# trailofbits/reverie

Measured on AMD Instinct MI355X. Metric: prover AND-gates/sec on GF(2) Bristol circuit; 1/2/4/8-GPU; proof bit-exact, higher is better.
Workload: dtype u32; 1 GPU; synthetic layered AND/XOR GF(2) circuit, 10027008 gates (5014185 AND), 4096 inputs, 153 layers x 65536, p_and=0.5, 256 reps x 8 players, 40 online; parallelism=reps/1, levels=163, compile_hint=RV_COMPILE_WHOLE_PROVER, gate_stream_bytes=334698564

## Files before the change

reverie_amd/csrc/batch.inc:

```

static int replay_recorded(rv_ctx* ctx, std::vector<LaunchRecorder>& recs, std::vector<void*>& pinned_tmp, std::vector<void*>& device_tmp) {
    const size_t batch = recs.size(), n = recs[0].calls.size();
    for (size_t b = 1; b < batch; b++)
        if (recs[b].calls.size() != n) return RV_E_DEVICE;
    size_t total = 0;
    std::vector<size_t> off(n, 0);
    for (size_t i = 0; i < n; i++) {
        const auto& c0 = recs[0].calls[i];
        for (size_t b = 1; b < batch; b++) {
            const auto& c = recs[b].calls[i];
            if (c.replay != c0.replay || c.fill != c0.fill || c.grid.x != c0.grid.x || c.block.x != c0.block.x || c.arg_bytes != c0.arg_bytes) return RV_E_DEVICE;
        }
        if (!c0.replay) continue;
        if (c0.grid.y != 1 || c0.grid.z != 1) return RV_E_DEVICE;
        off[i] = total;
        total += ((size_t)c0.arg_bytes * batch + 15) & ~(size_t)15;
    }
    uint8_t* d_args = nullptr;
    if (total) {
        uint8_t* h = (uint8_t*)g_pinned.get(std::max<size_t>(total, PinnedPool::MIN_BYTES));
        if (!h) return RV_E_NOMEM;
        pinned_tmp.push_back(h);
        for (size_t i = 0; i < n; i++) {
            const uint32_t ab = recs[0].calls[i].arg_bytes;
            if (!recs[0].calls[i].replay) continue;
            for (size_t b = 0; b < batch; b++) memcpy(h + off[i] + b * ab, recs[b].calls[i].args.data(), ab);
        }
        int r = dalloc(ctx, total, &d_args);
        if (r) return r;
        device_tmp.push_back(d_args);
        if (hipMemcpyAsync(d_args, h, total, hipMemcpyHostToDevice, ctx->stream) != hipSuccess) return RV_E_DEVICE;
    }
    for (size_t i = 0; i < n; i++) {
        const auto& c0 = recs[0].calls[i];
        if (c0.replay) {
            c0.replay(ctx->stream, c0.grid, c0.block, d_args + off[i], (unsigned)batch);
        } else {
            for (size_t b = 0; b < batch; b++) {
                const auto& c = recs[b].calls[i];
                if ((c.fill ? hipMemsetAsync(c.dst, c.value, c.n, ctx->stream) : hipMemcpyAsync(c.dst, c.src, c.n, c.kind, ctx->stream)) != hipSuccess)
                    return RV_E_DEVICE;
            }
        }
    }
    if (hipGetLastError() != hipSuccess) return RV_E_DEVICE;
    for (auto& r : recs) r.calls.clear();
    return RV_OK;
}

static size_t batch_big_gates() {
    static const size_t n = [] {
        const char* e = getenv("RV_BATCH_BIG_GATES");
        return e ? (size_t)strtoull(e, nullptr, 10) : (size_t)1 << 20;
    }();
    return n;
}

static void launch_levels_batched(rv_ctx* ctx, const rv_circuit* c, int mode, const InterpParams* d_pp, const Interp64Params* d_pp64, size_t batch) {
    const Compiled& cc = c->cc;
    const bool has64 = !cc.gates64.empty();
    const size_t n_levels = cc.level_start.empty() ? 0 : cc.level_start.size() - 1;
    for (size_t l = 0; l < n_levels; l++) {
        if (lds_run_for_batch(c, l, batch)) {
            const auto& pl = c->lds_runs[(size_t)c->lds_run_of_level[l]];
            if (l == pl.run.l0) {
                launch_interp_lds(ctx->stream, mode, pl.qs, RV_TOTAL_REPS / 4, c->d_lds_recs + pl.run.rec0, pl.run.n_steps, pl.run.n_slots,
                                  pl.run.eo0, pl.run.ep0, InterpParams{}, d_pp, (uint32_t)batch);
                if (has64) ctx->count();
            }
            continue;
        }
        if (c->run_of_level[l] >= 0) {
            const auto& run = c->narrow_runs[(size_t)c->run_of_level[l]];
            if (l == run.first) {
                launch_interp_narrow_batched(ctx->stream, c->d_gates, c->d_level_range, run.first, run.second, run.tiny, d_pp, (uint32_t)batch, mode);
                if (has64) ctx->count();
            }
            continue;
        }
        launch_interp_batched(ctx->stream, c->d_gates, cc.level_range[l], d_pp, (uint32_t)batch, mode);
        if (has64 && cc.level_start[l + 1] > cc.level_start[l]) ctx->count();
        if (has64 && cc.level_start64[l + 1] > cc.level_start64[l]) {
            launch_interp64_batched(ctx->stream, mode, c->d_gates64, cc.level_start64[l], cc.level_start64[l + 1], d_pp64, (uint32_t)batch);
            ctx->count();
        }
    }
}

struct BatchDst {
    uint8_t** proofs;
    size_t* proof_lens;
    uint8_t* d_dst;
    size_t stride;
};

static int prove_framed_device(rv_ctx* ctx, const rv_circuit* c, const WitSrc& w, const uint8_t* seeds, uint8_t* d_dst) {
    rv_shard* s = nullptr;
    int rc = rv_shard_commit_impl(ctx, c, w, seeds, 0, RV_TOTAL_REPS, &s, true);
    if (rc) return rc;
    do {
        void* d = nullptr;
        size_t lens[4];
        if ((rc = shard_open_impl(s, nullptr, d_dst, &d, lens, true, nullptr, nullptr, true))) break;
        int err = 0;
        if (!launch_frame_counts(ctx->stream, d_dst, 0, 1, lens) || hipGetLastError() != hipSuccess) {
            rc = RV_E_DEVICE;
            break;
        }
        if (hipMemcpyAsync(&err, s->d_err, sizeof err, hipMemcpyDeviceToHost, ctx->stream) != hipSuccess ||
            hipStreamSynchronize(ctx->stream) != hipSuccess) {
            rc = hip_fail(hipGetLastError(), "rv_prove_batch_device", __FILE__, __LINE__);
            break;
        }
        ctx->collect();
        if (err) rc = RV_E_WITNESS_INVALID;
    } while (0);
    rv_shard_destroy(s);
    return rc;
}

static int rv_prove_batch_impl(rv_ctx* ctx, const rv_circuit* c, size_t batch, const WitSrc& w, const uint8_t* seeds, const BatchDst& out) {
    LibBusy busy_guard;
    const uint8_t* const wit_gf2 = w.gf2;
    const uint64_t* const wit_z64 = w.z64;
    const size_t n_gf2 = w.n_gf2, n_z64 = w.n_z64;
    uint8_t** const proofs = out.proofs;
    size_t* const proof_lens = out.proof_lens;
    const bool dev = out.d_dst != nullptr;
    if (!ctx || !c || !batch || (dev ? !seeds : (!proofs || !proof_lens))) return RV_E_ARG;
    const Compiled& cc = c->cc;
    for (size_t b = 0; b < batch && !dev; b++) proofs[b] = nullptr, proof_lens[b] = 0;
    if (n_gf2 < cc.n_in || n_z64 < cc.n_in64) return RV_E_WITNESS_SHORT;
    if ((cc.n_in && !wit_gf2) || (cc.n_in64 && !wit_z64)) return RV_E_ARG;
    std::vector<uint8_t> os_seeds;
    if (!seeds) {
        os_seeds.resize(batch * RV_TOTAL_REPS * 16);
        size_t got = 0;
        while (got < os_seeds.size()) {
            ssize_t n = getrandom(os_seeds.data() + got, os_seeds.size() - got, 0);
            if (n <= 0) return RV_E_DEVICE;
            got += (size_t)n;
        }
        seeds = os_seeds.data();
    }
    auto one_by_one = [&]() {
        for (size_t b = 0; b < batch && dev; b++) {
            int rc = prove_framed_device(ctx, c, w.from(b), seeds + b * RV_TOTAL_REPS * 16, out.d_dst + b * out.stride);
            if (rc) return rc;
        }
        if (dev) return (int)RV_OK;
        for (size_t b = 0; b < batch; b++) {
            int rc = guarded([&]() -> int { return rv_prove_impl(ctx, c, w.from(b), seeds + b * RV_TOTAL_REPS * 16, &proofs[b], &proof_lens[b]); });
            if (rc) {
                for (size_t k = 0; k <= b; k++) rv_free(proofs[k]), proofs[k] = nullptr, proof_lens[k] = 0;
                return rc;
            }
        }
        return (int)RV_OK;
    };
    if (batch == 1) return one_by_one();
    HIPCHK(hipSetDevice(ctx->device));
    const size_t big_gates = batch_big_gates();
    const bool has64 = !cc.gates64.empty();
    if (has64 && cc.gates.size() + cc.gates64.size() >= big_gates) return one_by_one();
    if (has64) {
        size_t free_b = 0, total_b = 0;
        if (hipMemGetInfo(&free_b, &total_b) != hipSuccess) return RV_E_DEVICE;
        uint8_t om[RV_TOTAL_REPS];
        for (uint32_t r = 0; r < RV_TOTAL_REPS; r++) om[r] = r < RV_ONLINE_REPS ? 0 : RV_PLAYERS;
        const size_t per_proof = cc.info.scratch_bytes + open_layout(cc, om, RV_TOTAL_REPS, true).total + cc.n_in + 8 * cc.n_in64 + 4096;
        size_t chunk = std::min<size_t>(std::max<size_t>((free_b + ctx->cached_bytes) / 2 / per_proof, 2), 4096);
        if (const char* e = getenv("RV_BATCH_MAX")) chunk = std::min<size_t>(chunk, (size_t)std::max(atoi(e), 1));
        if (batch > chunk) {
            for (size_t b0 = 0; b0 < batch; b0 += chunk) {
                const int rc = rv_prove_batch_impl(ctx, c, std::min(chunk, batch - b0), w.from(b0), seeds + b0 * RV_TOTAL_REPS * 16,
                                                   dev ? BatchDst{nullptr, nullptr, out.d_dst + b0 * out.stride, out.stride}
                                                       : BatchDst{proofs + b0, proof_lens + b0, nullptr, 0});
                if (rc) {
                    for (size_t k = 0; k < b0 && !dev; k++) rv_free(proofs[k]), proofs[k] = nullptr, proof_lens[k] = 0;
                    return rc;
                }
            }
            return RV_OK;
        }
    }
    if (dev && cc.gates.size() >= big_gates) return one_by_one();
    if (cc.gates.size() >= big_gates) {
        constexpr size_t T_MAX = 8;
        static const size_t T = [] {
            const char* e = getenv("RV_BATCH_THREADS");
            return (size_t)std::min(std::max(e ? atoi(e) : 3, 1), (int)T_MAX);
        }();
        static const std::string classes = [] {
            const char* e = getenv("RV_BATCH_CLASSES");
            return std::string(e ? e : "HLHLHLHLHLHLHLHL");
        }();
        static const int prio_levels = [] {
            int lo = 0, hi = 0;
            if (hipDeviceGetStreamPriorityRange(&lo, &hi) != hipSuccess) lo = hi = 0, (void)hipGetLastError();
            return lo - hi + 1;
        }();
        auto cls = [&](size_t i) {
            const char ch = i < classes.size() ? classes[i] : 'N';
            const int lowest = prio_levels - 1;
            return prio_levels < 2 ? -1 : ch == 'H' ? 0 : ch == 'L' ? lowest : lowest / 2 + (lowest == 1 ? -1 : 0);
        };
        while (ctx->workers.size() < T) {
            rv_ctx* w = nullptr;
            const size_t k = ctx->workers.size();
            int mc = cls(2 * k), kc = cls(2 * k + 1);
            if (mc < 0 && kc >= 0) mc = kc;
            int rcw = ctx_create_impl(ctx->device, &w, mc, kc);
            if (rcw) return rcw;
            ctx->workers.push_back(w);
        }
        uint8_t canon[RV_TOTAL_REPS];
        for (uint32_t r = 0; r < RV_TOTAL_REPS; r++) canon[r] = r < RV_ONLINE_REPS ? 0 : RV_PLAYERS;
        const size_t stride = (open_layout(cc, canon, RV_TOTAL_REPS, true).total + 4095) & ~(size_t)4095;
        uint8_t* slab = (uint8_t*)g_pinned.get(std::max<size_t>(stride * batch, PinnedPool::MIN_BYTES));
        if (!slab) return RV_E_NOMEM;
        int rcs[T_MAX] = {};
        std::thread th[T_MAX];
        static const bool big_stats = getenv("RV_BATCH_STATS") != nullptr;
        const auto t_call = std::chrono::steady_clock::now();
        std::vector<std::array<double, 5>> span(batch);
        std::atomic<size_t> next_proof{0};
        for (size_t t = 0; t < T; t++)
            th[t] = std::thread([&, t] {
                try {
                    if (hipSetDevice(ctx->device) != hipSuccess) {
                        rcs[t] = RV_E_DEVICE;
                        return;
                    }
                    for (size_t b; rcs[t] == RV_OK && (b = next_proof.fetch_add(1, std::memory_order_relaxed)) < batch;) {
                        span[b][0] = std::chrono::duration<double, std::milli>(std::chrono::steady_clock::now() - t_call).count();
                        rcs[t] = rv_prove_impl(ctx->workers[t], c, WitSrc{w.from(b).gf2, n_gf2, w.stride_gf2, nullptr, 0, 0, w.dev},
                                               seeds + b * RV_TOTAL_REPS * 16, &proofs[b], &proof_lens[b], slab + b * stride, stride);
                        span[b][1] = std::chrono::duration<double, std::milli>(std::chrono::steady_clock::now() - t_call).count();
                        for (int k = 0; k < 3; k++) span[b][2 + k] = g_prove_marks[k];
                        if (big_stats && g_prove_marks[1] > 5.0) {
                            std::string line = "[rv batch] slow host side, proof " + std::to_string(b) + ":";
                            for (auto& m : g_ht.marks) line += std::string(" ") + m.first + " " + std::to_string(m.second).substr(0, 5);
                            fprintf(stderr, "%s\n", line.c_str());
                        }
                    }
                } catch (...) {
                    rcs[t] = RV_E_NOMEM;
                }
            });
        for (size_t t = 0; t < T; t++) th[t].join();
        if (big_stats) {
            fprintf(stderr, "[rv batch] %zu proofs on %zu workers, %.2f ms:", batch, T,
                    std::chrono::duration<double, std::milli>(std::chrono::steady_clock::now() - t_call).count());
            for (size_t b = 0; b < batch; b++)
                fprintf(stderr, " %zu[%.1f-%.1f: q %.1f o %.1f s %.1f]", b, span[b][0], span[b][1], span[b][2], span[b][3], span[b][4]);
            fprintf(stderr, "\n");
        }
        for (int r : rcs)
            if (r) {
                for (size_t b = 0; b < batch; b++) proofs[b] = nullptr, proof_lens[b] = 0;
                g_pinned.put(slab);
                return r;
            }
        g_pinned.share(slab, batch);
        ctx->prof.calls += batch;
        return RV_OK;
    }
    std::vector<rv_shard*> sh(batch, nullptr);
    std::vector<InterpParams> pp(batch);
    std::vector<Interp64Params> pp64(has64 ? batch : 0);
    InterpParams* d_pp = nullptr;
    int rc = RV_OK;
    uint8_t* staging = nullptr;
    std::vector<void*> pinned_tmp;
    std::vector<void*> device_tmp;
    auto cleanup = [&](int code) {
        g_recorder = nullptr;
        (void)hipStreamSynchronize(ctx->stream);
        for (rv_shard* s : sh)
            if (s) {
                s->destroy();
                delete s;
            }
        ctx->release(d_pp);
        for (void* q : device_tmp) ctx->release(q);
        for (void* q : pinned_tmp) g_pinned.put(q);
        if (staging) g_pinned.put(staging);
        if (code && !dev)
            for (size_t b = 0; b < batch; b++) rv_free(proofs[b]), proofs[b] = nullptr, proof_lens[b] = 0;
        return code;
    };
    const uint32_t R = RV_TOTAL_REPS;
    std::vector<LaunchRecorder> recs(batch);
    for (auto& r : recs) r.batch = (unsigned)batch;
    struct RecorderOff {
        ~RecorderOff() { g_recorder = nullptr; }
    } recorder_off;
    static const bool stats = getenv("RV_BATCH_STATS") != nullptr;
    auto t_last = std::chrono::steady_clock::now();
    auto mark = [&](const char* what) {
        if (!stats) return;
        const auto t = std::chrono::steady_clock::now();
        fprintf(stderr, "[rv batch] %-28s %8.3f ms\n", what, std::chrono::duration<double, std::milli>(t - t_last).count());
        t_last = t;
    };
    auto replay = [&]() -> int { return replay_recorded(ctx, recs, pinned_tmp, device_tmp); };
    constexpr size_t SLAB_HEAD = 256;
    const size_t wit_stride = (std::max<size_t>(cc.n_in, 1) + 15) & ~(size_t)15;
    uint8_t canon[RV_TOTAL_REPS];
    for (uint32_t r = 0; r < RV_TOTAL_REPS; r++) canon[r] = r < RV_ONLINE_REPS ? 0 : RV_PLAYERS;
    const size_t out_stride = (open_layout(cc, canon, R, true).total + 4 + 255) & ~(size_t)255;
    uint8_t *d_seeds_all = nullptr, *d_wit_all = nullptr, *d_out_all = nullptr;
    int* d_err_all = nullptr;
    if ((rc = dalloc(ctx, SLAB_HEAD + batch * (size_t)R * 16, &d_seeds_all))) return cleanup(rc);
    device_tmp.push_back(d_seeds_all);
    if ((rc = dalloc(ctx, SLAB_HEAD + batch * wit_stride, &d_wit_all))) return cleanup(rc);
    device_tmp.push_back(d_wit_all);
    if (!dev) {
        if ((rc = dalloc(ctx, SLAB_HEAD + batch * out_stride, &d_out_all))) return cleanup(rc);
        device_tmp.push_back(d_out_all);
    }
    if ((rc = dalloc(ctx, SLAB_HEAD / sizeof(int) + batch, &d_err_all))) return cleanup(rc);
    device_tmp.push_back(d_err_all);
    if (hipMemcpyAsync(d_seeds_all + SLAB_HEAD, seeds, batch * (size_t)R * 16, hipMemcpyHostToDevice, ctx->stream) != hipSuccess ||
        (cc.n_in && hipMemcpy2DAsync(d_wit_all + SLAB_HEAD, wit_stride, wit_gf2, w.stride_gf2, cc.n_in, batch, w.kind(),
                                     ctx->stream) != hipSuccess))
        return cleanup(RV_E_DEVICE);
    const size_t wit64_stride = (std::max<size_t>(cc.n_in64, 1) + 1) & ~(size_t)1;
    uint64_t* d_wit64_all = nullptr;
    if (has64) {
        if ((rc = dalloc(ctx, SLAB_HEAD / 8 + batch * wit64_stride, &d_wit64_all))) return cleanup(rc);
        device_tmp.push_back(d_wit64_all);
        if (cc.n_in64 && hipMemcpy2DAsync(d_wit64_all + SLAB_HEAD / 8, wit64_stride * 8, wit_z64, w.stride_z64 * 8, cc.n_in64 * 8, batch,
                                          w.kind(), ctx->stream) != hipSuccess)
            return cleanup(RV_E_DEVICE);
    }
    wit_count(w, batch * (cc.n_in + cc.n_in64 * 8));
    for (size_t b = 0; b < batch && !rc; b++) {
        rv_shard* s = sh[b] = new rv_shard();
        s->ctx = ctx;
        s->c = c;
        s->rep_begin = 0;
        s->R = R;
        s->NQ = R / 4;
        s->d_seeds = d_seeds_all + SLAB_HEAD + b * (size_t)R * 16;
        s->d_wit = d_wit_all + SLAB_HEAD + b * wit_stride;
        s->d_err = d_err_all + SLAB_HEAD / sizeof(int) + b;
        if ((rc = dalloc(ctx, (size_t)R * 128, &s->d_keys))) break;
        g_recorder = &recs[b];
        launch_expand_seeds(ctx->stream, s->d_seeds, R, s->d_keys);
        Interp64Params p64{};
        pp[b] = InterpParams{};
        pp[b].wit = s->d_wit;
        if (!(rc = shard_setup_prg(s, nullptr))) rc = shard_run_alloc(s, pp[b], p64);
        if (has64) {
            p64.wit = d_wit64_all + SLAB_HEAD / 8 + b * wit64_stride;
            pp64[b] = p64;
        }
        g_recorder = nullptr;
    }
    if (rc) return cleanup(rc);
    mark("record setup/masks");
    ctx->phase(RV_PH_MASKS);
    if ((rc = replay())) return cleanup(rc);
    mark("replay setup/masks");
    ctx->phase(RV_PH_INTERP);
    if ((rc = dalloc(ctx, batch, &d_pp))) return cleanup(rc);
    if (hipMemcpyAsync(d_pp, pp.data(), batch * sizeof(InterpParams), hipMemcpyHostToDevice, ctx->stream) != hipSuccess) return cleanup(RV_E_DEVICE);
    Interp64Params* d_pp64 = nullptr;
    if (has64) {
        if ((rc = dalloc(ctx, batch, &d_pp64))) return cleanup(rc);
        device_tmp.push_back(d_pp64);
        if (hipMemcpyAsync(d_pp64, pp64.data(), batch * sizeof(Interp64Params), hipMemcpyHostToDevice, ctx->stream) != hipSuccess) return cleanup(RV_E_DEVICE);
    }
    launch_levels_batched(ctx, c, MODE_PROVE, d_pp, d_pp64, batch);
    if (has64) ctx->phase(-1);
    mark("interpreter launches");
    size_t slot = 0;
    size_t lens[4] = {0, 0, 0, 0};
    for (size_t b = 0; b < batch && !rc; b++) {
        rv_shard* s = sh[b];
        void* d = nullptr;
        g_recorder = &recs[b];
        if (!(rc = shard_run_hash(s)) && !(rc = shard_join(s)))
            rc = shard_open_impl(s, nullptr, dev ? out.d_dst + b * out.stride : d_out_all + SLAB_HEAD + b * out_stride, &d, lens, true, nullptr, nullptr, true);
        g_recorder = nullptr;
    }
    if (rc) return cleanup(rc);
    mark("record digests/openings");
    ctx->phase(RV_PH_HASH);
    if ((rc = replay())) return cleanup(rc);
    ctx->phase(-1);
    mark("replay digests/openings");
    const size_t total = 32 + 4 * 8 + lens[0] + lens[1] + lens[2] + lens[3];
    if (dev) {
        if (total > out.stride || batch > 0x3FFFFFFFu || !launch_frame_counts(ctx->stream, out.d_dst, out.stride, (uint32_t)batch, lens) ||
            hipGetLastError() != hipSuccess)
            return cleanup(RV_E_DEVICE);
        staging = (uint8_t*)g_pinned.get(std::max<size_t>(batch * sizeof(int), PinnedPool::MIN_BYTES));
        if (!staging) return cleanup(RV_E_NOMEM);
        if (hipMemcpyAsync(staging, d_err_all + SLAB_HEAD / sizeof(int), batch * sizeof(int), hipMemcpyDeviceToHost, ctx->stream) != hipSuccess)
            return cleanup(RV_E_DEVICE);
    } else {
        if (total > out_stride) return cleanup(RV_E_DEVICE);
        slot = out_stride;
        staging = (uint8_t*)g_pinned.get(std::max<size_t>(slot * batch + batch * sizeof(int), PinnedPool::MIN_BYTES));
        if (!staging) return cleanup(RV_E_NOMEM);
        if (hipMemcpyAsync(staging, d_out_all + SLAB_HEAD, slot * batch, hipMemcpyDeviceToHost, ctx->stream) != hipSuccess ||
            hipMemcpyAsync(staging + slot * batch, d_err_all + SLAB_HEAD / sizeof(int), batch * sizeof(int), hipMemcpyDeviceToHost,
                           ctx->stream) != hipSuccess)
            return cleanup(RV_E_DEVICE);
        for (size_t b = 0; b < batch; b++) proof_lens[b] = total;
    }
    mark("queue device-to-host copies");
    if (hipStreamSynchronize(ctx->stream) != hipSuccess) return cleanup(hip_fail(hipGetLastError(), "batch sync", __FILE__, __LINE__));
    ctx->collect();
    mark("wait for the GPU");
    for (size_t b = 0; b < batch; b++) {
        int err = 0;
        memcpy(&err, staging + slot * batch + b * sizeof(int), sizeof err);
        if (err) return cleanup(RV_E_WITNESS_INVALID);
    }
    if (!dev) {
        static const bool copy_out = getenv("RV_BATCH_COPY_OUT") != nullptr;
        const uint64_t counts[4] = {RV_ONLINE_REPS, RV_PREPROCESSING_REPS, RV_ONLINE_REPS, RV_PREPROCESSING_REPS};
        if (copy_out) {
            for (size_t b = 0; b < batch; b++) {
                proofs[b] = (uint8_t*)malloc(proof_lens[b]);
                if (!proofs[b]) return cleanup(RV_E_NOMEM);
                memcpy(proofs[b], staging + b * slot, proof_lens[b]);
            }
        } else {
            g_pinned.share(staging, batch);
            for (size_t b = 0; b < batch; b++) proofs[b] = staging + b * slot;
            staging = nullptr;
        }
        for (size_t b = 0; b < batch; b++) {
            size_t off = 32;
            for (int k = 0; k < 4; k++) {
                put_le64(proofs[b] + off, counts[k]);
                off += 8 + lens[k];
            }
        }
    }
    ctx->prof.calls += batch;
    mark("copy proofs out");
    rc = cleanup(RV_OK);
    mark("cleanup");
    return rc;
}

extern "C" int rv_prove_batch(rv_ctx* ctx, const rv_circuit* c, size_t batch, const uint8_t* wit_gf2, size_t n_gf2,
                              const uint64_t* wit_z64, size_t n_z64, const uint8_t* seeds, uint8_t** proofs, size_t* proof_lens) {
    try {
        return rv_prove_batch_impl(ctx, c, batch, wit_host(wit_gf2, n_gf2, wit_z64, n_z64), seeds, BatchDst{proofs, proof_lens, nullptr, 0});
    } catch (...) {
        g_last_error = "out of host memory";
        return RV_E_NOMEM;
    }
}
```

reverie_amd/csrc/gf2dev.h:

```cpp
#pragma once
#include <hip/hip_runtime.h>
#include <stdint.h>

namespace rv {

__device__ __forceinline__ uint32_t smear01(uint32_t t) {
    uint32_t r;
    asm("v_lshlrev_b32 %0, 8, %1\n\tv_sub_u32 %0, %0, %1" : "=&v"(r) : "v"(t));
    return r;
}
__device__ __forceinline__ uint32_t recon32(uint32_t t) {
    t ^= t >> 4;
    t ^= t >> 2;
    t ^= t >> 1;
    t &= 0x01010101u;
    return smear01(t);
}

__device__ __forceinline__ uint32_t expand4(uint32_t n) {
    const uint32_t t = (n | (n << 7) | (n << 14) | (n << 21)) & 0x01010101u;
    return smear01(t);
}
__device__ __forceinline__ uint32_t compress4(uint32_t x) {
    const uint32_t y = x & 0x08040201u;
    return (y | (y >> 8) | (y >> 16) | (y >> 24)) & 0xFu;
}
__device__ __forceinline__ uint32_t load_bits(const uint8_t* base, size_t row, uint32_t NQ, uint32_t q) {
    return expand4(((uint32_t)base[row * (NQ >> 1) + (q >> 1)] >> (4 * (q & 1))) & 0xFu);
}
__device__ __forceinline__ uint32_t pair_swap(uint32_t v) {
    return (uint32_t)__builtin_amdgcn_mov_dpp((int)v, 0xB1, 0xF, 0xF, true);
}
__device__ __forceinline__ void store_bits(uint8_t* base, size_t row, uint32_t NQ, uint32_t q, uint32_t smeared) {
    const uint32_t n = compress4(smeared);
    const uint32_t other = pair_swap(n);
    if (!(q & 1)) base[row * (NQ >> 1) + (q >> 1)] = (uint8_t)(n | (other << 4));
}

}
```

reverie_amd/csrc/internal.h:

```cpp
#pragma once
#include <hip/hip_runtime.h>
#include <stddef.h>
#include <stdint.h>

#include "../../include/reverie_amd.h"

namespace rv {


constexpr int RV_LIN_K = 3;
struct Gate {
    uint32_t op;
    uint32_t dst;
    uint32_t m;
    uint32_t eo;
    uint32_t ep;
    uint32_t x;
    uint32_t a[RV_LIN_K], b[RV_LIN_K];
};

enum GateOp : uint32_t {
    G_INPUT = 0,
    G_XORK,
    G_MUL,
    G_ASSERT,
    G_RANDOM,
    G_RECON
};
__host__ __device__ inline uint32_t g_op(const Gate& g) { return g.op & 0xFFu; }
__host__ __device__ inline uint32_t g_na(const Gate& g) { return (g.op >> 8) & 0xFu; }
__host__ __device__ inline uint32_t g_nb(const Gate& g) { return (g.op >> 12) & 0xFu; }
__host__ __device__ inline uint32_t g_ca(const Gate& g) { return (g.op >> 16) & 1u; }
__host__ __device__ inline uint32_t g_cb(const Gate& g) { return (g.op >> 17) & 1u; }

struct Gate64 {
    uint32_t op;
    uint32_t dst;
    uint32_t a, b;
    uint32_t m;
    uint32_t m2;
    uint64_t eo;
    uint64_t ep;
    uint32_t x;
    uint32_t xc;
    uint64_t imm;
    uint32_t am, bm;
};
constexpr uint32_t G64_MASK_ROW = 0x80000000u;

enum Gate64Op : uint32_t {
    G64_INPUT = 0, G64_ADD, G64_SUB, G64_ADDC, G64_SUBC, G64_MULC, G64_MUL, G64_ASSERT, G64_RANDOM, G64_CONST, G64_B2A
};

struct Interp64Params {
    uint32_t R;
    uint64_t* wmask;
    uint64_t* wcorr;
    const uint64_t* masks;
    uint64_t* on;
    uint64_t* pre;
    uint64_t on_words, pre_words;
    const uint64_t* wit;
    const uint8_t* omit;
    const uint64_t* sup_in;
    const uint64_t* sup_corr;
    const uint64_t* sup_rec;
    uint32_t sup_r;
    const uint8_t* corr2;
    const uint32_t* masks2;
    uint32_t NQ;
    int* err;
};

enum Mode : int { MODE_PROVE = 0, MODE_VERIFY = 1, MODE_PROVE_V = 2, MODE_VERIFY_C = 4 };
constexpr int RV_DEV_ZERO_CHECK = 0x100;

struct InterpParams {
    uint32_t NQ;
    uint32_t* rows;
    uint8_t* corr;
    uint32_t* on;
    uint8_t* pre;
    uint8_t* vclr;
    uint64_t* vc;
    const uint8_t* wit;
    const uint32_t* on_mask;
    const uint32_t* sup_in;
    const uint32_t* sup_corr;
    const uint32_t* sup_rec;
    uint32_t sup_nq;
    int* err;
};

void set_device_lds_limit(size_t bytes);
size_t device_lds_limit();

struct EvalParams {
    uint32_t B, W;
    uint32_t* val;
    const uint32_t* win;
    uint64_t* v64;
    const uint64_t* wz;
    uint64_t wz_stride;
    uint32_t* n_failed;
    uint32_t* first2;
    uint32_t* first64;
};
struct WireForm {
    uint32_t b[RV_LIN_K];
    uint32_t c;
};
void launch_eval_level(hipStream_t st, const EvalParams& p, const Gate* d_gates, uint32_t lo, uint32_t n2, const Gate64* d_gates64, uint32_t lo64,
                       uint32_t n64);
struct LevelRange;
void launch_eval_walk(hipStream_t st, const EvalParams& p, const Gate* d_gates, const LevelRange* d_lr, const Gate64* d_gates64, const uint32_t* d_ls64,
                      uint32_t n_levels, uint32_t S, uint32_t threads);
void launch_eval_wit(hipStream_t st, const uint8_t* d_wit , size_t stride, uint32_t n, uint32_t B, uint32_t W,
                     uint32_t* d_out );
void launch_eval_out(hipStream_t st, const EvalParams& p, const WireForm* d_forms, uint32_t n_gf2, const uint32_t* d_ssa64, uint32_t n_z64,
                     uint8_t* d_out2 , uint64_t* d_out64 );

struct EvalFold {
    const uint32_t* rec2;
    const uint64_t* op2;
    const uint32_t* rec64;
    const uint64_t* op64;
    uint32_t n2, n64;
    uint64_t op_base;
    uint64_t* first_op;
    uint64_t* total;
};
void launch_eval_fold(hipStream_t st, const EvalParams& p, const EvalFold& f);
void launch_eval_out_sel(hipStream_t st, const EvalParams& p, const WireForm* d_forms, const uint32_t* d_sel2, uint32_t n_sel2, const uint32_t* d_ssa64,
                         const uint32_t* d_sel64, uint32_t n_sel64, uint8_t* d_out2 , uint64_t* d_out64 );
void launch_eval_status(hipStream_t st, const EvalParams& p, const EvalFold& f, rv_eval_status* d_out );
void launch_eval_stream_out(hipStream_t st, const EvalParams& p, uint32_t n_gf2, uint32_t n_z64, uint32_t b0, uint32_t nb, uint8_t* d_out2,
                            uint64_t* d_out64);

void launch_expand_seeds(hipStream_t st, const uint8_t* d_seeds, uint32_t n_reps, uint8_t* d_keys );
constexpr uint32_t RK_BYTES = 208;
constexpr uint32_t RK_AREAS = 13;
constexpr uint64_t RV_MAX_CTR_BLOCKS = 1ull << 24;
void launch_key_schedule(hipStream_t st, const uint8_t* d_keys, uint32_t n_slots, uint8_t* d_rkbytes );
void launch_setup_keys(hipStream_t st, const uint8_t* d_seeds, uint32_t NQ, uint8_t* d_keys, uint8_t* d_rkbytes, uint32_t* d_rk, uint32_t* d_img);
void launch_bitslice_rk(hipStream_t st, const uint8_t* d_rkbytes, uint32_t NQ, uint32_t* d_rk );
void launch_aes_gf2_masks(hipStream_t st, const uint32_t* d_rk, const uint32_t* d_keep, uint32_t NQ, uint64_t first_block,
                          uint64_t n_blocks, uint32_t* d_masks);
bool aes_col4_supports(uint32_t NQ);
size_t aes_col4_image_bytes(uint32_t NQ);
void launch_rk_col4(hipStream_t st, const uint32_t* d_rk, uint32_t NQ, uint32_t* d_img);
void launch_aes_gf2_masks_col4(hipStream_t st, const uint32_t* d_img, const uint32_t* d_keep, uint32_t NQ, uint64_t first_block, uint64_t n_blocks,
                               uint32_t* d_masks);
void launch_aes_blocks(hipStream_t st, const uint8_t* d_rkbytes, uint32_t n_keys, uint64_t first_block, uint64_t n_blocks,
                       uint8_t* d_out);
struct LevelRange {
    uint32_t lo, mul11, mul, xor2, xork, hi;
};
bool any_level_general(const LevelRange* lr, size_t n_levels);
void launch_interp(hipStream_t st, int mode, const Gate* d_gates, const LevelRange& r, const InterpParams& p,
                   const LevelRange* next = nullptr);
void launch_interp_narrow(hipStream_t st, int mode, const Gate* d_gates, const LevelRange* d_level_range, uint32_t l0, uint32_t l1,
                          int tiny, const InterpParams& p);
void launch_interp_batched(hipStream_t st, const Gate* d_gates, const LevelRange& r, const InterpParams* d_pp, uint32_t batch,
                           int mode = MODE_PROVE);
bool b3_pair_big_ok(uint64_t n_pre, uint64_t n_on, uint32_t NQ, const uint32_t* d_quads = nullptr, uint32_t n_quads = 0);
uint32_t launch_b3_pair_big(hipStream_t st, const uint8_t* d_pre, uint64_t n_pre, const uint32_t* d_on, uint64_t n_on, uint32_t NQ, uint32_t* cv_a0,
                            uint32_t* cv_a1, uint32_t* cv_b0, uint32_t* cv_b1, uint32_t* d_dig_pre, uint32_t* d_dig_on, const uint32_t* d_quads = nullptr,
                            uint32_t n_quads = 0);
bool launch_b3_pair_small(hipStream_t st, const uint8_t* d_pre, uint64_t n_pre, const uint32_t* d_on, uint64_t n_on, uint32_t NQ, uint32_t* d_cv_a,
                          uint32_t* d_cv_b, uint32_t* d_dig_pre, uint32_t* d_dig_on, const uint32_t* d_quads = nullptr, uint32_t n_quads = 0);
void launch_store_word(hipStream_t st, const int* d_src, int* dst_mapped);
void launch_pack_corr_all(hipStream_t st, const uint8_t* d_bits, uint64_t n_items, uint64_t byte0, uint64_t n_bytes, uint64_t pitch, uint8_t* d_out);
struct OpenDirect {
    uint32_t n_direct = 0, tile = 0;
    uint64_t rvec_at = 0, rvec_len = 0;
};
void launch_copy_gaps(hipStream_t st, const uint8_t* d_img, uint8_t* dst_mapped, uint64_t total, uint64_t first, uint64_t rec, uint64_t corr_at,
                      uint64_t corr_len, uint32_t n_rec, const uint8_t* d_omit , uint32_t rep_limit, OpenDirect od = OpenDirect(),
                      const int* d_err = nullptr, int* err_dst_mapped = nullptr );
uint32_t extract_tile_bytes(uint64_t n_items);
uint32_t extract_from_bits_tile_bytes(uint64_t n_items);
void launch_publish(hipStream_t st, const uint32_t* d_src, uint32_t n_words, uint32_t* dst_mapped, uint32_t* flag_mapped, uint32_t seq);
void launch_store_words(hipStream_t st, const uint32_t* d_src, uint32_t n_words, uint32_t* dst_mapped, const int* d_err, int* dst_err_mapped);
bool launch_frame_counts(hipStream_t st, uint8_t* d_out, uint64_t stride, uint32_t batch, const size_t lens[4]);
struct LdsRec;
void launch_interp_lds(hipStream_t st, int mode, uint32_t QS, uint32_t NQ, const LdsRec* d_recs, uint32_t n_steps, uint32_t n_slots,
                       uint32_t eo0, uint32_t ep0, const InterpParams& p, const InterpParams* d_pp, uint32_t batch);
void launch_interp_narrow_batched(hipStream_t st, const Gate* d_gates, const LevelRange* d_level_range, uint32_t l0, uint32_t l1,
                                  int tiny, const InterpParams* d_pp, uint32_t batch, int mode = MODE_PROVE);
void launch_interp64(hipStream_t st, int mode, const Gate64* d_gates, uint32_t lo, uint32_t hi, const Interp64Params& p);
void launch_interp64_batched(hipStream_t st, int mode, const Gate64* d_gates, uint32_t lo, uint32_t hi, const Interp64Params* d_pp, uint32_t batch);
void launch_aes_z64_masks(hipStream_t st, const uint32_t* d_rk, const uint32_t* d_keep, uint32_t NQ, uint64_t n_blocks,
                          uint64_t* d_masks64, uint64_t first_block = 0);
struct Z64FLevel {
    uint32_t mul0, mul1, lin1, oth1;
};
struct Z64FParams {
    const uint32_t* rk;
    uint32_t NQ;
    uint64_t* wmask;
    uint64_t* masks;
    uint64_t* on;
    uint64_t* pre;
    uint64_t on_words, pre_words;
    const uint64_t* wit;
    uint64_t* v;
    int* err;
    uint64_t first_block;
    uint32_t qg0, qgn;
    const uint8_t* omit;
    const uint32_t* keep;
    uint64_t* wcorr;
    const uint64_t* sup_in;
    const uint64_t* sup_corr;
    const uint64_t* sup_rec;
    uint32_t sup_r;
};
bool z64_fused_supports(uint32_t NQ);
uint32_t z64_fused_qw(uint32_t NQ);
void launch_z64_fused(hipStream_t st, const Gate64* d_gates, const Z64FLevel& lv, const Z64FParams& p);
uint32_t launch_b3_contig(hipStream_t st, const uint64_t* d_streams, uint64_t n_words, uint32_t R, uint32_t* d_cv_a, uint32_t* d_cv_b,
                      uint32_t* d_digest);
void launch_extract64(hipStream_t st, const uint64_t* d_stream, uint64_t stride_words, const uint64_t* d_offs ,
                      uint64_t n_items, int add_omit, uint32_t R, const uint8_t* d_omit, const uint64_t* d_dst_off, uint8_t* d_out,
                      const struct OnlineList* d_ol = nullptr ,
                      uint32_t rep_min = 0 );
void launch_unpack64(hipStream_t st, const uint8_t* d_blob, const uint64_t* d_src_off, const uint64_t* d_src_len,
                     const uint8_t* d_omit, uint64_t n_items, uint32_t R, uint64_t* d_out, uint32_t out_r );
uint32_t launch_b3_stream(hipStream_t st, const uint32_t* d_stream, uint64_t n_events, uint32_t NQ, uint32_t* d_cv_a,
                      uint32_t* d_cv_b, uint32_t* d_digest , const uint32_t* d_quads = nullptr, uint32_t n_quads = 0);
uint32_t launch_b3_stream_bits(hipStream_t st, const uint8_t* d_stream, uint64_t n_events, uint32_t NQ, uint32_t* d_cv_a,
                           uint32_t* d_cv_b, uint32_t* d_digest);
size_t b3_stream_scratch_words(uint64_t n_events, uint32_t R);
void launch_b3_stream_chunks(hipStream_t st, const uint32_t* d_stream, uint64_t n_events, uint32_t NQ, uint32_t* d_cv, const uint32_t* d_quads,
                             uint32_t n_quads, uint64_t chunk_base, uint32_t root_ok);
void launch_b3_stream_bits_chunks(hipStream_t st, const uint8_t* d_stream, uint64_t n_events, uint32_t NQ, uint32_t* d_cv, uint64_t chunk_base,
                                  uint32_t root_ok);
void launch_b3_contig_chunks(hipStream_t st, const uint64_t* d_streams, uint64_t stride_words, uint64_t n_words, uint32_t R, uint32_t* d_cv,
                             uint64_t chunk_base, uint32_t root_ok);
void launch_b3_pairs(hipStream_t st, const uint32_t* d_pending, const uint32_t* d_in, uint64_t n_pairs, uint32_t R, uint32_t* d_out);
struct B3PairsBatch {
    static constexpr uint32_t MAX = 32;
    const uint32_t* pending[MAX];
    const uint32_t* in[MAX];
    uint32_t* out[MAX];
    uint32_t n;
};
void launch_b3_pairs_batched(hipStream_t st, const B3PairsBatch& L, uint64_t n_pairs, uint32_t R);
struct B3FoldList {
    uint32_t n;
    const uint32_t* p[48];
};
void launch_b3_fold(hipStream_t st, const B3FoldList& L, const uint32_t* d_last, uint32_t R, uint32_t* d_digest);
uint32_t b3_reduce_tree(hipStream_t st, uint32_t* cur, uint32_t* nxt, uint64_t n, uint32_t R, uint32_t* d_digest);
void launch_join(hipStream_t st, const uint32_t* d_pre2, const uint32_t* d_on2, const uint32_t* d_pre64, const uint32_t* d_on64,
                 uint32_t R, uint8_t* d_h );
struct OnlineList {
    uint32_t n;
    uint32_t rep[RV_ONLINE_REPS];
    uint64_t dst[RV_ONLINE_REPS];
};
void launch_extract_from_bits(hipStream_t st, const uint8_t* d_bits, uint64_t n_items, uint32_t NQ,
                              const OnlineList* d_ol , uint8_t* d_out, uint32_t rep_min = 0 );
struct FsLayout {
    uint64_t base[4];
    uint64_t sz2, sz64, l2r, l2c, l64r, l64c;
    uint32_t framed;
    uint8_t* comm2;
};
void launch_fs_challenge(hipStream_t st, const uint8_t* d_h, const FsLayout& L, uint32_t rep_begin, uint32_t R, uint8_t* d_comm,
                         uint8_t* d_omit, uint8_t* d_omit_all, uint64_t* d_offs, OnlineList* d_ol, uint32_t* d_res,
                         uint32_t* mbox = nullptr ,
                         uint32_t* mbox_flag = nullptr, uint32_t mbox_seq = 0);
bool launch_open_small(hipStream_t st, uint32_t R, const uint8_t* d_omit, const uint8_t* d_seeds, const uint8_t* d_keys, const uint32_t* d_on2,
                       const uint32_t* d_on64, const uint64_t* d_offs, uint64_t l2r, uint64_t l2c, uint64_t l2i, uint64_t l64r, uint64_t l64c, uint64_t l64i,
                       const uint32_t* d_on, const uint32_t* d_rec_rows, uint64_t n_rec, const uint8_t* d_pre, uint64_t n_pre, const uint32_t* d_in_rows,
                       uint64_t n_in, uint32_t NQ, const OnlineList* d_ol, uint32_t corr_rep_min, uint8_t* d_out, const int* d_err, int* err_dst_mapped,
                       bool heads_inputs_only = false);
void launch_extract_bits(hipStream_t st, const void* d_stream, const uint32_t* d_rows , uint64_t n_items,
                         uint32_t NQ, int kind, const uint8_t* d_omit, const uint64_t* d_dst_off, uint8_t* d_out, uint8_t* d_out2 = nullptr,
                         uint32_t n_direct = 0);
void launch_unpack_bits(hipStream_t st, const uint8_t* d_blob, const uint64_t* d_src_off, const uint64_t* d_src_len,
                        const uint8_t* d_omit, uint64_t n_items, uint32_t NQ, int kind, uint32_t* d_rows_out, uint32_t out_nq ,
                        uint64_t first_item = 0 );
void launch_shard_init(hipStream_t st, int* d_err, uint32_t* d_zero_mask, uint32_t n_mask_words , uint8_t* d_zero_corr,
                       uint32_t n_corr_bytes , uint32_t* d_fill = nullptr , uint32_t n_fill_rows = 0,
                       const uint32_t* digest = nullptr, uint8_t* d_zero_byte = nullptr );
void launch_fill_digests(hipStream_t st, uint32_t* d_dst, uint32_t n_rows, const uint32_t digest[8]);
void launch_overlay_rows(hipStream_t st, uint32_t* d_dst, const uint32_t* d_src, const uint8_t* d_omit, uint32_t R,
                         uint32_t row_words, int want_online);
void launch_hook_recon_gf2(hipStream_t st, const uint64_t* d_shares, uint64_t n, uint64_t* d_out);
void launch_hook_recon_z64(hipStream_t st, const uint64_t* d_shares , uint64_t n, uint64_t* d_out );
void launch_open_headers(hipStream_t st, uint32_t R, const uint8_t* d_omit, const uint8_t* d_seeds, const uint8_t* d_keys,
                         const uint32_t* d_on2, const uint32_t* d_on64, const uint64_t* d_off2, const uint64_t* d_off64,
                         uint64_t lens2_rec, uint64_t lens2_corr, uint64_t lens2_in, uint64_t lens64_rec, uint64_t lens64_corr,
                         uint64_t lens64_in, uint8_t* d_out);


}
```

reverie_amd/csrc/interp.hip:

```cpp
#include <stdlib.h>

#include <algorithm>

#include "gf2dev.h"
#include "internal.h"
#include "launch.h"

namespace rv {

static size_t g_device_lds_limit = 160 * 1024;
void set_device_lds_limit(size_t bytes) { g_device_lds_limit = bytes; }
size_t device_lds_limit() { return g_device_lds_limit; }


__device__ __forceinline__ uint32_t gather_rows(const uint32_t* rows, const uint32_t* ids, uint32_t NQ, uint32_t q) {
    uint32_t v = 0;
#pragma unroll
    for (int i = 0; i < RV_LIN_K; i++) v ^= rows[(size_t)ids[i] * NQ + q];
    return v;
}
__device__ __forceinline__ uint32_t gather_corr_byte(const uint8_t* corr, const uint32_t* ids, uint32_t NQ, uint32_t o) {
    uint32_t v = 0;
#pragma unroll
    for (int i = 0; i < RV_LIN_K; i++) v ^= corr[(size_t)ids[i] * (NQ >> 1) + o];
    return v;
}
__device__ __forceinline__ uint32_t gather_corr(const uint8_t* corr, const uint32_t* ids, uint32_t NQ, uint32_t q) {
    return (gather_corr_byte(corr, ids, NQ, q >> 1) >> (4 * (q & 1))) & 0xFu;
}

__device__ __forceinline__ uint32_t gather_vclr(const uint8_t* vclr, const uint32_t* ids) {
    uint32_t v = 0;
#pragma unroll
    for (int i = 0; i < RV_LIN_K; i++) v ^= vclr[ids[i]];
    return v;
}

__device__ __forceinline__ uint32_t vc_nib(uint64_t c, uint32_t q) {
    const uint32_t w = (q & 8) ? (uint32_t)(c >> 32) : (uint32_t)c;
    return q < 16 ? (w >> (4 * (q & 7))) & 0xFu : 0u;
}
__device__ __forceinline__ uint64_t gather_vc(const uint64_t* vc, const uint32_t* ids) {
    uint64_t v = 0;
#pragma unroll
    for (int i = 0; i < RV_LIN_K; i++) v ^= vc[ids[i]];
    return v;
}
__device__ __forceinline__ void vc_store(uint64_t* vc, size_t row, uint32_t q, uint32_t smeared) {
    uint32_t v = q < 16 ? compress4(smeared) << (4 * (q & 7)) : 0u;
    v |= (uint32_t)__builtin_amdgcn_update_dpp(0, (int)v, 0x111, 0xF, 0xF, true);
    v |= (uint32_t)__builtin_amdgcn_update_dpp(0, (int)v, 0x112, 0xF, 0xF, true);
    v |= (uint32_t)__builtin_amdgcn_update_dpp(0, (int)v, 0x114, 0xF, 0xF, true);
    if (q == 7 || q == 15) ((uint32_t*)(vc + row))[q >> 3] = v;
}
constexpr bool is_verify(int mode) { return mode == MODE_VERIFY || mode == MODE_VERIFY_C; }

template <int MODE>
__device__ __forceinline__ void interp_one(const Gate& g, const InterpParams& p, uint32_t NQ, uint32_t q, uint32_t onm) {
    switch (g_op(g)) {
    case G_INPUT: {
        const uint32_t lam = p.rows[(size_t)g.m * NQ + q];
        uint32_t corr;
        if (!is_verify(MODE)) {
            const uint32_t w = p.wit[g.x] ? 0xFFFFFFFFu : 0u;
            corr = w ^ recon32(lam);
        } else {
            corr = onm ? (p.sup_in[(size_t)g.x * p.sup_nq + q] & onm) : 0u;
        }
        if (!is_verify(MODE) || onm) p.on[(size_t)g.eo * NQ + q] = corr;
        if (MODE == MODE_PROVE_V) {
            if (q == 0) p.vclr[g.dst] = p.wit[g.x] ? 1 : 0;
        } else if (MODE == MODE_VERIFY_C) {
            vc_store(p.vc, g.dst, q, corr);
        } else {
            store_bits(p.corr, g.dst, NQ, q, corr);
        }
        break;
    }
    case G_XORK: {
        p.rows[(size_t)g.dst * NQ + q] = gather_rows(p.rows, g.a, NQ, q) ^ gather_rows(p.rows, g.b, NQ, q);
        if (MODE == MODE_PROVE_V) {
            if (q == 0) p.vclr[g.dst] = (uint8_t)((g_ca(g) ^ gather_vclr(p.vclr, g.a) ^ gather_vclr(p.vclr, g.b)) & 1u);
            break;
        }
        if (MODE == MODE_VERIFY_C) {
            if (q == 0) p.vc[g.dst] = gather_vc(p.vc, g.a) ^ gather_vc(p.vc, g.b) ^ (g_ca(g) ? ~0ull : 0ull);
            break;
        }
        if (!(q & 1)) {
            const size_t h = NQ >> 1, o = q >> 1;
            const uint32_t c = (g_ca(g) ? 0xFFu : 0u) ^ gather_corr_byte(p.corr, g.a, NQ, o) ^ gather_corr_byte(p.corr, g.b, NQ, o);
            p.corr[(size_t)g.dst * h + o] = (uint8_t)c;
        }
        break;
    }
    case G_RANDOM: {
        if (MODE == MODE_VERIFY_C) {
            if (q == 0) p.vc[g.dst] = 0;
            break;
        }
        if (!(q & 1)) p.corr[(size_t)g.dst * (NQ >> 1) + (q >> 1)] = 0;
        break;
    }
    case G_MUL: {
        const uint32_t lx = gather_rows(p.rows, g.a, NQ, q), ly = gather_rows(p.rows, g.b, NQ, q);
        const uint32_t lab = p.rows[(size_t)g.m * NQ + q], lnew = p.rows[(size_t)(g.m + 1) * NQ + q];
        const uint32_t a = recon32(lx), b = recon32(ly), c = recon32(lab);
        uint32_t cx, cy, vx = 0, vy = 0;
        if (MODE == MODE_PROVE_V) {
            vx = (gather_vclr(p.vclr, g.a) ^ g_ca(g)) & 1u;
            vy = (gather_vclr(p.vclr, g.b) ^ g_cb(g)) & 1u;
            cx = a ^ (vx ? 0xFFFFFFFFu : 0u);
            cy = b ^ (vy ? 0xFFFFFFFFu : 0u);
        } else if (MODE == MODE_VERIFY_C) {
            cx = expand4(vc_nib(gather_vc(p.vc, g.a), q)) ^ (g_ca(g) ? 0xFFFFFFFFu : 0u);
            cy = expand4(vc_nib(gather_vc(p.vc, g.b), q)) ^ (g_cb(g) ? 0xFFFFFFFFu : 0u);
        } else {
            cx = expand4(gather_corr(p.corr, g.a, NQ, q)) ^ (g_ca(g) ? 0xFFFFFFFFu : 0u);
            cy = expand4(gather_corr(p.corr, g.b, NQ, q)) ^ (g_cb(g) ? 0xFFFFFFFFu : 0u);
        }
        uint32_t delta = (a & b) ^ c;
        uint32_t s = (ly & cx) ^ (lx & cy) ^ lab ^ lnew;
        uint32_t r;
        if (!is_verify(MODE)) {
            r = recon32(s);
        } else {
            if (onm) {
                delta = (p.sup_corr[(size_t)g.ep * p.sup_nq + q] & onm) | (delta & ~onm);
                s ^= p.sup_rec[(size_t)g.x * p.sup_nq + q];
            }
            r = recon32(s) & onm;
        }
        if (!is_verify(MODE) || onm) p.on[(size_t)g.eo * NQ + q] = s;
        store_bits(p.pre, g.ep, NQ, q, delta);
        if (MODE == MODE_PROVE_V) {
            if (q == 0) p.vclr[g.dst] = (uint8_t)(vx & vy);
        } else if (MODE == MODE_VERIFY_C) {
            vc_store(p.vc, g.dst, q, r ^ delta ^ (cx & cy));
        } else {
            store_bits(p.corr, g.dst, NQ, q, r ^ delta ^ (cx & cy));
        }
        break;
    }
    case G_RECON: {
        uint32_t m = gather_rows(p.rows, g.a, NQ, q);
        if (is_verify(MODE) && onm) m ^= p.sup_rec[(size_t)g.x * p.sup_nq + q];
        if (MODE == MODE_PROVE || onm) p.on[(size_t)g.eo * NQ + q] = m;
        uint32_t r = recon32(m);
        if (is_verify(MODE)) r &= onm;
        const uint32_t cx = expand4(gather_corr(p.corr, g.a, NQ, q)) ^ (g_ca(g) ? 0xFFFFFFFFu : 0u);
        p.rows[(size_t)g.dst * NQ + q] = 0;
        store_bits(p.corr, g.dst, NQ, q, r ^ cx);
        break;
    }
    case G_ASSERT: {
        uint32_t m = gather_rows(p.rows, g.a, NQ, q);
        if (is_verify(MODE) && onm) m ^= p.sup_rec[(size_t)g.x * p.sup_nq + q];
        if (!is_verify(MODE) || onm) p.on[(size_t)g.eo * NQ + q] = m;
        if (MODE == MODE_PROVE_V) {
            if (q == 0 && ((gather_vclr(p.vclr, g.a) ^ g_ca(g)) & 1u) != 0) atomicOr(p.err, RV_E_WITNESS_INVALID);
        } else {
            const uint32_t cx = expand4(MODE == MODE_VERIFY_C ? vc_nib(gather_vc(p.vc, g.a), q) : gather_corr(p.corr, g.a, NQ, q)) ^ (g_ca(g) ? 0xFFFFFFFFu : 0u);
            if (MODE == MODE_PROVE) {
                if ((recon32(m) ^ cx) != 0) atomicOr(p.err, RV_E_WITNESS_INVALID);
            } else {
                if (((recon32(m) ^ cx) & onm) != 0) atomicOr(p.err, RV_DEV_ZERO_CHECK);
            }
        }
        break;
    }
    default:
        break;
    }
}

template <int MODE>
__global__ __launch_bounds__(256) void k_interp(const Gate* __restrict__ gates, uint32_t lo, uint32_t hi, InterpParams p) {
    const uint32_t NQ = p.NQ;
    const uint32_t tid = blockIdx.x * blockDim.x + threadIdx.x;
    const uint32_t q = tid % NQ;
    const uint32_t worker = tid / NQ;
    const uint32_t n_workers = (gridDim.x * blockDim.x) / NQ;
    const uint32_t onm = (is_verify(MODE)) ? p.on_mask[q] : 0u;
    for (uint32_t gi = lo + worker; gi < hi; gi += n_workers) {
        const Gate g = gates[gi];
        interp_one<MODE>(g, p, NQ, q, onm);
    }
}

#ifndef RV_INTERP_UNROLL
#define RV_INTERP_UNROLL 4
#endif
#ifndef RV_INTERP_UNROLL_SMALL
#define RV_INTERP_UNROLL_SMALL 2
#endif
#ifndef RV_INTERP_UNROLL_MID
#define RV_INTERP_UNROLL_MID 4
#endif
#ifndef RV_INTERP_UNROLL_FAST
#define RV_INTERP_UNROLL_FAST 4
#endif
#ifndef RV_INTERP_UXOR_FAST
#define RV_INTERP_UXOR_FAST 0
#endif
__host__ __device__ constexpr int interp_unroll(int NQ, bool general = true) {
    return NQ >= 64 ? (general ? RV_INTERP_UNROLL : RV_INTERP_UNROLL_FAST) : NQ >= 32 ? RV_INTERP_UNROLL_MID : RV_INTERP_UNROLL_SMALL;
}

struct PfPlan {
    uint32_t dist;
    uint32_t rem;
    uint32_t n[2][4];
    uint32_t start[2][4];
};
template <uint32_t STEP>
__device__ __forceinline__ const Gate* pf_target(const Gate* __restrict__ gates, const PfPlan& pf, uint32_t t) {
    uint32_t tt = t + pf.dist;
#pragma unroll
    for (int k = 0; k < 2; k++) {
#pragma unroll
        for (int c = 0; c < 4; c++) {
            if (tt < pf.n[k][c]) return gates + pf.start[k][c] + tt * STEP;
            tt -= pf.n[k][c];
        }
        tt += pf.rem;
    }
    return nullptr;
}
template <uint32_t STEP>
__device__ __forceinline__ uint32_t pf_touch(const Gate* g, uint32_t lane) {
    constexpr uint32_t BYTES = STEP * (uint32_t)sizeof(Gate), NL = (BYTES + 127) / 128;
    uint32_t v = 0;
    if (g && lane <= NL) v = *(const uint32_t*)((const char*)g + (lane < NL ? lane * 128 : BYTES - 4));
    return v;
}
__device__ __forceinline__ void pf_sink(uint32_t v) { asm volatile("" ::"v"(v)); }

template <int MODE, int NQ, int U, int KA, int KB>
__device__ __forceinline__ void mulU(const Gate* __restrict__ gates, uint32_t g0, const InterpParams& p, uint32_t sub, uint32_t q,
                                     uint32_t onm, const Gate* pf = nullptr) {
    constexpr uint32_t GPW = 64 / NQ, H = NQ / 2;
    const bool on_wr = !is_verify(MODE) || ((__ballot(onm != 0) >> ((sub * NQ + q) & ~7u)) & 0xFFull) != 0;
    Gate g[U];
#pragma unroll
    for (int u = 0; u < U; u++) g[u] = gates[g0 + u * GPW + sub];
    uint32_t lx[U], ly[U], lab[U], lnew[U], bx[U], by[U], sc[U], sr[U];
    uint32_t ra[U][KA], ca[U][KA], rb[U][KB], cb[U][KB];
    const uint32_t* const vc32 = (const uint32_t*)p.vc + ((q >> 3) & 1u);
#pragma unroll
    for (int u = 0; u < U; u++) {
        const int na = (int)g_na(g[u]), nb = (int)g_nb(g[u]);
#pragma unroll
        for (int i = 0; i < KA; i++) {
            ra[u][i] = 0;
            ca[u][i] = 0;
            if (i == 0 || i < na) {
                ra[u][i] = p.rows[(size_t)g[u].a[i] * NQ + q];
                ca[u][i] = MODE == MODE_VERIFY_C ? vc32[2 * (size_t)g[u].a[i]]
                                                 : MODE == MODE_PROVE_V ? p.vclr[g[u].a[i]] : p.corr[(size_t)g[u].a[i] * H + (q >> 1)];
            }
        }
#pragma unroll
        for (int i = 0; i < KB; i++) {
            rb[u][i] = 0;
            cb[u][i] = 0;
            if (i == 0 || i < nb) {
                rb[u][i] = p.rows[(size_t)g[u].b[i] * NQ + q];
                cb[u][i] = MODE == MODE_VERIFY_C ? vc32[2 * (size_t)g[u].b[i]]
                                                 : MODE == MODE_PROVE_V ? p.vclr[g[u].b[i]] : p.corr[(size_t)g[u].b[i] * H + (q >> 1)];
            }
        }
        lab[u] = __builtin_nontemporal_load(&p.rows[(size_t)g[u].m * NQ + q]);
        lnew[u] = p.rows[(size_t)(g[u].m + 1) * NQ + q];
        if (is_verify(MODE)) {
            sc[u] = sr[u] = 0;
            if (onm) {
                sc[u] = p.sup_corr[(size_t)g[u].ep * p.sup_nq + q];
                sr[u] = p.sup_rec[(size_t)g[u].x * p.sup_nq + q];
            }
        }
    }
    const uint32_t pfv = pf_touch<U * GPW>(pf, sub * NQ + q);
#pragma unroll
    for (int u = 0; u < U; u++) {
        lx[u] = ra[u][0];
        bx[u] = ca[u][0];
        ly[u] = rb[u][0];
        by[u] = cb[u][0];
#pragma unroll
        for (int i = 1; i < KA; i++) {
            lx[u] ^= ra[u][i];
            bx[u] ^= ca[u][i];
        }
#pragma unroll
        for (int i = 1; i < KB; i++) {
            ly[u] ^= rb[u][i];
            by[u] ^= cb[u][i];
        }
    }
#pragma unroll
    for (int u = 0; u < U; u++) {
        const uint32_t a = recon32(lx[u]), b = recon32(ly[u]), c = recon32(lab[u]);
        uint32_t cx, cy;
        const uint32_t vx = (bx[u] ^ g_ca(g[u])) & 1u, vy = (by[u] ^ g_cb(g[u])) & 1u;
        if (MODE == MODE_PROVE_V) {
            cx = a ^ (vx ? 0xFFFFFFFFu : 0u);
            cy = b ^ (vy ? 0xFFFFFFFFu : 0u);
        } else if (MODE == MODE_VERIFY_C) {
            cx = expand4(q < 16 ? (bx[u] >> (4 * (q & 7))) & 0xFu : 0u) ^ (g_ca(g[u]) ? 0xFFFFFFFFu : 0u);
            cy = expand4(q < 16 ? (by[u] >> (4 * (q & 7))) & 0xFu : 0u) ^ (g_cb(g[u]) ? 0xFFFFFFFFu : 0u);
        } else {
            cx = expand4((bx[u] >> (4 * (q & 1))) & 0xFu) ^ (g_ca(g[u]) ? 0xFFFFFFFFu : 0u);
            cy = expand4((by[u] >> (4 * (q & 1))) & 0xFu) ^ (g_cb(g[u]) ? 0xFFFFFFFFu : 0u);
        }
        uint32_t delta = (a & b) ^ c;
        uint32_t s = (ly[u] & cx) ^ (lx[u] & cy) ^ lab[u] ^ lnew[u];
        uint32_t r = 0;
        if (MODE == MODE_PROVE) {
            r = recon32(s);
        } else if (is_verify(MODE)) {
            delta = (sc[u] & onm) | (delta & ~onm);
            s ^= sr[u];
            r = recon32(s) & onm;
        }
        if (!is_verify(MODE) || on_wr) __builtin_nontemporal_store(s, &p.on[(size_t)g[u].eo * NQ + q]);
        store_bits(p.pre, g[u].ep, NQ, q, delta);
        if (MODE == MODE_PROVE_V) {
            if (q == 0) p.vclr[g[u].dst] = (uint8_t)(vx & vy);
        } else if (MODE == MODE_VERIFY_C) {
            vc_store(p.vc, g[u].dst, q, r ^ delta ^ (cx & cy));
        } else {
            store_bits(p.corr, g[u].dst, NQ, q, r ^ delta ^ (cx & cy));
        }
    }
    pf_sink(pfv);
}

template <int MODE, int NQ, int U, int N>
__device__ __forceinline__ void xorU(const Gate* __restrict__ gates, uint32_t g0, const InterpParams& p, uint32_t sub, uint32_t q,
                                     const Gate* pf = nullptr) {
    constexpr uint32_t GPW = 64 / NQ, H = NQ / 2;
    Gate g[U];
#pragma unroll
    for (int u = 0; u < U; u++) g[u] = gates[g0 + u * GPW + sub];
    uint32_t x[U], bx[U], rr[U][N], cc[U][N];
#pragma unroll
    for (int u = 0; u < U; u++) {
        const int na = (int)g_na(g[u]), nb = (int)g_nb(g[u]);
#pragma unroll
        for (int i = 0; i < N; i++) {
            const uint32_t id = (N == 2) ? g[u].a[i] : (i < RV_LIN_K ? g[u].a[i] : g[u].b[i - RV_LIN_K]);
            rr[u][i] = 0;
            cc[u][i] = 0;
            if (N == 2 || (i < RV_LIN_K ? i < na : i - RV_LIN_K < nb)) {
                rr[u][i] = p.rows[(size_t)id * NQ + q];
                if (MODE == MODE_PROVE_V) {
                    if (q == 0) cc[u][i] = p.vclr[id];
                } else if (MODE == MODE_VERIFY_C) {
                    if (q < 2) cc[u][i] = ((const uint32_t*)p.vc)[2 * (size_t)id + q];
                } else if (q < H) {
                    cc[u][i] = p.corr[(size_t)id * H + q];
                }
            }
        }
    }
    const uint32_t pfv = pf_touch<U * GPW>(pf, sub * NQ + q);
#pragma unroll
    for (int u = 0; u < U; u++) {
        x[u] = 0;
        bx[u] = 0;
#pragma unroll
        for (int i = 0; i < N; i++) {
            x[u] ^= rr[u][i];
            bx[u] ^= cc[u][i];
        }
    }
#pragma unroll
    for (int u = 0; u < U; u++) {
        p.rows[(size_t)g[u].dst * NQ + q] = x[u];
        if (MODE == MODE_PROVE_V) {
            if (q == 0) p.vclr[g[u].dst] = (uint8_t)((bx[u] ^ g_ca(g[u])) & 1u);
        } else if (MODE == MODE_VERIFY_C) {
            if (q < 2) ((uint32_t*)p.vc)[2 * (size_t)g[u].dst + q] = bx[u] ^ (g_ca(g[u]) ? 0xFFFFFFFFu : 0u);
        } else if (q < H) {
            p.corr[(size_t)g[u].dst * H + q] = (uint8_t)(bx[u] ^ (g_ca(g[u]) ? 0xFFu : 0u));
        }
    }
    pf_sink(pfv);
}

template <int MODE, int NQ, bool GENERAL = true, bool PF = false, int UXOR = 0>
__device__ __forceinline__ void run_level(const Gate* __restrict__ gates, const LevelRange& r, const InterpParams& p, uint32_t wave,
                                          uint32_t n_waves, uint32_t lane, uint32_t onm, const Gate* pf_gates = nullptr,
                                          const PfPlan* pf = nullptr) {
    constexpr uint32_t GPW = 64 / NQ;
    const uint32_t q = lane % NQ, sub = lane / NQ;
    constexpr int U = interp_unroll(NQ, GENERAL);
    constexpr int UX = UXOR ? UXOR : U;
    static_assert(!PF || UX == U, "the prefetch plan assumes one step size");
    uint32_t slot = 0;
    auto my = [&](uint32_t used) { return (wave + n_waves - used % n_waves) % n_waves; };
    const uint32_t begin[5] = {r.lo, r.mul11, r.mul, r.xor2, r.xork}, end[5] = {r.mul11, r.mul, r.xor2, r.xork, r.hi};
    uint32_t rest[5];
#pragma unroll
    for (int c = 0; c < 4; c++) {
        const uint32_t STEP = (uint32_t)(c >= 2 ? UX : U) * GPW;
        const uint32_t n_full = (!GENERAL && (c == 1 || c == 3)) ? 0u : (end[c] - begin[c]) / STEP;
        rest[c] = begin[c] + n_full * STEP;
        for (uint32_t g0 = begin[c] + my(slot) * STEP; g0 < rest[c]; g0 += n_waves * STEP) {
            const Gate* t = nullptr;
            if (PF && pf->dist) t = pf_target<U * GPW>(pf_gates, *pf, slot + (g0 - begin[c]) / STEP);
            if (c == 0) mulU<MODE, NQ, U, 1, 1>(gates, g0, p, sub, q, onm, t);
            if (c == 1 && GENERAL) mulU<MODE, NQ, U, RV_LIN_K, RV_LIN_K>(gates, g0, p, sub, q, onm, t);
            if (c == 2) xorU<MODE, NQ, UX, 2>(gates, g0, p, sub, q, t);
            if (c == 3 && GENERAL) xorU<MODE, NQ, UX, 2 * RV_LIN_K>(gates, g0, p, sub, q, t);
        }
        slot += n_full;
    }
    rest[4] = begin[4];
    uint32_t cum[6];
    cum[0] = 0;
#pragma unroll
    for (int c = 0; c < 5; c++) cum[c + 1] = cum[c] + (end[c] - rest[c] + GPW - 1) / GPW;
    for (uint32_t t = my(slot); t < cum[5]; t += n_waves) {
        uint32_t c0 = rest[0], e0 = end[0], base = 0;
#pragma unroll
        for (int c = 1; c < 5; c++)
            if (t >= cum[c]) c0 = rest[c], e0 = end[c], base = cum[c];
        const uint32_t gi = c0 + (t - base) * GPW + sub;
        if (gi < e0) interp_one<MODE>(gates[gi], p, NQ, q, onm);
    }
}

template <int MODE, int NQ, bool GENERAL>
__global__ __launch_bounds__(256, MODE == MODE_VERIFY_C ? (GENERAL ? 4 : 7) : (GENERAL || NQ != 64) ? 1 : 8) void k_interp_full(const Gate* __restrict__ gates, LevelRange r, InterpParams p, PfPlan pf) {
    __builtin_amdgcn_s_setprio(1);
    const uint32_t lane = threadIdx.x & 63;
    const uint32_t wave = __builtin_amdgcn_readfirstlane((blockIdx.x * blockDim.x + threadIdx.x) >> 6);
    const uint32_t n_waves = gridDim.x * (blockDim.x >> 6);
    const uint32_t onm = (is_verify(MODE)) ? p.on_mask[lane % NQ] : 0u;
    constexpr int UXL = (!GENERAL && NQ == 64) ? RV_INTERP_UXOR_FAST : 0;
    constexpr bool PFL = UXL == 0 || UXL == interp_unroll(NQ, GENERAL);
    run_level<MODE, NQ, GENERAL, PFL, UXL>(gates, r, p, wave, n_waves, lane, onm, gates, &pf);
}

template <int MODE, int NQ>
__global__ __launch_bounds__(256) void k_interp_full_b(const Gate* __restrict__ gates, LevelRange r, const InterpParams* __restrict__ pp) {
    const InterpParams p = pp[blockIdx.y];
    const uint32_t lane = threadIdx.x & 63;
    const uint32_t wave = __builtin_amdgcn_readfirstlane((blockIdx.x * blockDim.x + threadIdx.x) >> 6);
    const uint32_t n_waves = gridDim.x * (blockDim.x >> 6);
    const uint32_t onm = (is_verify(MODE)) ? p.on_mask[lane % NQ] : 0u;
    run_level<MODE, NQ>(gates, r, p, wave, n_waves, lane, onm);
}

static bool level_is_general(const LevelRange& r) { return (r.mul - r.mul11) + (r.xork - r.xor2) >= 64; }

static uint32_t pf_dist(int NQ) {
    static const int env = [] {
        const char* e = getenv("RV_PF_DIST");
        return e ? atoi(e) : -1;
    }();
    const uint32_t v = env >= 0 ? (uint32_t)env : (NQ == 64 ? 4096u : 0u);
    return v & ~31u;
}

template <int NQ>
static PfPlan make_pf_plan(const LevelRange& r, const LevelRange* next) {
    constexpr uint32_t GPW = 64 / NQ;
    PfPlan pf{};
    pf.dist = pf_dist(NQ);
    if (!pf.dist) return pf;
    const LevelRange* lr[2] = {&r, next};
    uint32_t total = 0;
    for (int k = 0; k < 2; k++) {
        if (!lr[k]) break;
        const LevelRange& x = *lr[k];
        const bool general = level_is_general(x);
        const uint32_t step = (uint32_t)interp_unroll(NQ, general) * GPW;
        const uint32_t begin[4] = {x.lo, x.mul11, x.mul, x.xor2}, end[4] = {x.mul11, x.mul, x.xor2, x.xork};
        for (int c = 0; c < 4; c++) {
            pf.start[k][c] = begin[c];
            pf.n[k][c] = (!general && (c == 1 || c == 3)) ? 0u : (end[c] - begin[c]) / step;
            if (k == 0) total += pf.n[k][c];
        }
    }
    pf.rem = total & 31u;
    return pf;
}

template <int MODE, int NQ>
static void launch_interp_full_mode(hipStream_t st, dim3 grid, bool general, const Gate* d_gates, const LevelRange& r, const InterpParams& p,
                                    const PfPlan& pf) {
    if (general)
        hipLaunchKernelGGL((k_interp_full<MODE, NQ, true>), grid, dim3(256), 0, st, d_gates, r, p, pf);
    else
        hipLaunchKernelGGL((k_interp_full<MODE, NQ, false>), grid, dim3(256), 0, st, d_gates, r, p, pf);
}

template <int NQ>
static void launch_interp_full(hipStream_t st, int mode, const Gate* d_gates, const LevelRange& r, const InterpParams& p,
                               const LevelRange* next) {
    constexpr uint32_t GPW = 64 / NQ;
    const bool general = level_is_general(r);
    const PfPlan pf = make_pf_plan<NQ>(r, next);
    const uint32_t u = (uint32_t)interp_unroll(NQ, general);
    uint64_t waves = ((uint64_t)(r.hi - r.lo) + u * GPW - 1) / (u * GPW);
    uint64_t blocks = (waves + 3) / 4;
    if (blocks > 4096) blocks = 4096;
    if (blocks < 1) blocks = 1;
    const dim3 grid((unsigned)blocks);
    if (mode == MODE_PROVE_V) return launch_interp_full_mode<MODE_PROVE_V, NQ>(st, grid, general, d_gates, r, p, pf);
    if (mode == MODE_PROVE) return launch_interp_full_mode<MODE_PROVE, NQ>(st, grid, general, d_gates, r, p, pf);
    if constexpr (NQ == 64)
        if (mode == MODE_VERIFY_C) return launch_interp_full_mode<MODE_VERIFY_C, NQ>(st, grid, general, d_gates, r, p, pf);
    launch_interp_full_mode<MODE_VERIFY, NQ>(st, grid, general, d_gates, r, p, pf);
}


bool any_level_general(const LevelRange* lr, size_t n_levels) {
    for (size_t l = 0; l < n_levels; l++)
        if (level_is_general(lr[l])) return true;
    return false;
}

constexpr uint32_t NARROW_MAX_LEVELS = 1024;
constexpr uint32_t NARROW_WIN = 1024;
template <int MODE, int NQT, bool LEAN = false>
__device__ __forceinline__ void interp_narrow_body(const Gate* __restrict__ gates, const LevelRange* __restrict__ level_range,
                                                   uint32_t l0, uint32_t l1, const InterpParams& p) {
    __shared__ LevelRange s_lr[NARROW_MAX_LEVELS];
    __shared__ __attribute__((aligned(16))) Gate s_g[NARROW_WIN];
    const uint32_t NQ = NQT ? (uint32_t)NQT : p.NQ;
    const uint32_t lane = threadIdx.x & 63, wave = threadIdx.x >> 6;
    const uint32_t onm = (is_verify(MODE)) ? p.on_mask[NQT ? lane % NQ : threadIdx.x % NQ] : 0u;
    const uint32_t n_lv = l1 - l0;
    {
        const uint32_t* src = (const uint32_t*)(level_range + l0);
        uint32_t* dst = (uint32_t*)s_lr;
        for (uint32_t i = threadIdx.x; i < n_lv * (uint32_t)(sizeof(LevelRange) / 4); i += 1024) dst[i] = src[i];
    }
    __syncthreads();
    const uint32_t g_end = s_lr[n_lv - 1].hi;
    uint32_t win_lo = s_lr[0].lo, win_hi = win_lo;
    for (uint32_t l = 0; l < n_lv; l++) {
        const LevelRange r = s_lr[l];
        if (r.hi > win_hi) {
            win_lo = r.lo;
            win_hi = (r.lo + NARROW_WIN < g_end) ? r.lo + NARROW_WIN : g_end;
            const uint4* src = (const uint4*)(gates + win_lo);
            uint4* dst = (uint4*)s_g;
            for (uint32_t i = threadIdx.x; i < (win_hi - win_lo) * (uint32_t)(sizeof(Gate) / 16); i += 1024) dst[i] = src[i];
            __syncthreads();
        }
        const Gate* g = s_g - win_lo;
        if (NQT) {
            if (LEAN)
                run_level<MODE, NQT ? NQT : 64, false, false, 8>(g, r, p, wave, 16, lane, onm);
            else
                run_level<MODE, NQT ? NQT : 64>(g, r, p, wave, 16, lane, onm);
        } else {
            const uint32_t q = threadIdx.x % NQ, worker = threadIdx.x / NQ, n_workers = 1024 / NQ;
            for (uint32_t gi = r.lo + worker; gi < r.hi; gi += n_workers) interp_one<MODE>(g[gi], p, NQ, q, onm);
        }
        __syncthreads();
    }
}

template <int MODE, int NQT, bool LEAN = false>
__global__ __launch_bounds__(1024) void k_interp_narrow(const Gate* __restrict__ gates, const LevelRange* __restrict__ level_range,
                                                        uint32_t l0, uint32_t l1, InterpParams p) {
    interp_narrow_body<MODE, NQT, LEAN>(gates, level_range, l0, l1, p);
}
template <int MODE, int NQT>
__global__ __launch_bounds__(1024) void k_interp_narrow_b(const Gate* __restrict__ gates, const LevelRange* __restrict__ level_range,
                                                          uint32_t l0, uint32_t l1, const InterpParams* __restrict__ pp) {
    const InterpParams p = pp[blockIdx.x];
    interp_narrow_body<MODE, NQT>(gates, level_range, l0, l1, p);
}

template <int NQT, bool LEAN = false>
static void launch_narrow_nq(hipStream_t st, int mode, const Gate* d_gates, const LevelRange* d_lr, uint32_t a, uint32_t b,
                             const InterpParams& p) {
    if (mode == MODE_PROVE)
        hipLaunchKernelGGL((k_interp_narrow<MODE_PROVE, NQT, LEAN>), dim3(1), dim3(1024), 0, st, d_gates, d_lr, a, b, p);
    else
        hipLaunchKernelGGL((k_interp_narrow<MODE_VERIFY, NQT, LEAN>), dim3(1), dim3(1024), 0, st, d_gates, d_lr, a, b, p);
}

void launch_interp_narrow(hipStream_t st, int mode, const Gate* d_gates, const LevelRange* d_level_range, uint32_t l0, uint32_t l1,
                          int tiny, const InterpParams& p) {
    for (uint32_t a = l0; a < l1; a += NARROW_MAX_LEVELS) {
        const uint32_t b = (a + NARROW_MAX_LEVELS < l1) ? a + NARROW_MAX_LEVELS : l1;
        switch (tiny == 1 ? 0u : p.NQ) {
        case 64:
            if (tiny == 2)
                launch_narrow_nq<64, true>(st, mode, d_gates, d_level_range, a, b, p);
            else
                launch_narrow_nq<64>(st, mode, d_gates, d_level_range, a, b, p);
            break;
        case 32: launch_narrow_nq<32>(st, mode, d_gates, d_level_range, a, b, p); break;
        case 16: launch_narrow_nq<16>(st, mode, d_gates, d_level_range, a, b, p); break;
        case 8: launch_narrow_nq<8>(st, mode, d_gates, d_level_range, a, b, p); break;
        default: launch_narrow_nq<0>(st, mode, d_gates, d_level_range, a, b, p); break;
        }
    }
}

void launch_interp(hipStream_t st, int mode, const Gate* d_gates, const LevelRange& r, const InterpParams& p, const LevelRange* next) {
    if (r.hi <= r.lo) return;
    switch (p.NQ) {
    case 64: return launch_interp_full<64>(st, mode, d_gates, r, p, next);
    case 32: return launch_interp_full<32>(st, mode, d_gates, r, p, next);
    case 16: return launch_interp_full<16>(st, mode, d_gates, r, p, next);
    case 8: return launch_interp_full<8>(st, mode, d_gates, r, p, next);
    default: break;
    }
    const uint64_t want = (uint64_t)(r.hi - r.lo) * p.NQ;
    uint64_t blocks = (want + 255) / 256;
    if (blocks > 8192) blocks = 8192;
    if (mode == MODE_PROVE)
        hipLaunchKernelGGL(k_interp<MODE_PROVE>, dim3((unsigned)blocks), dim3(256), 0, st, d_gates, r.lo, r.hi, p);
    else
        hipLaunchKernelGGL(k_interp<MODE_VERIFY>, dim3((unsigned)blocks), dim3(256), 0, st, d_gates, r.lo, r.hi, p);
}

void launch_interp_batched(hipStream_t st, const Gate* d_gates, const LevelRange& r, const InterpParams* d_pp, uint32_t batch, int mode) {
    if (r.hi <= r.lo || !batch) return;
    uint64_t waves = ((uint64_t)(r.hi - r.lo) + RV_INTERP_UNROLL - 1) / RV_INTERP_UNROLL;
    uint64_t blocks = (waves + 3) / 4;
    const uint64_t cap = std::max<uint64_t>(4096 / batch, 1);
    if (blocks > cap) blocks = cap;
    if (mode == MODE_PROVE)
        hipLaunchKernelGGL((k_interp_full_b<MODE_PROVE, 64>), dim3((unsigned)blocks, batch), dim3(256), 0, st, d_gates, r, d_pp);
    else
        hipLaunchKernelGGL((k_interp_full_b<MODE_VERIFY, 64>), dim3((unsigned)blocks, batch), dim3(256), 0, st, d_gates, r, d_pp);
}

void launch_interp_narrow_batched(hipStream_t st, const Gate* d_gates, const LevelRange* d_level_range, uint32_t l0, uint32_t l1,
                                  int tiny, const InterpParams* d_pp, uint32_t batch, int mode) {
    for (uint32_t a = l0; a < l1 && batch; a += NARROW_MAX_LEVELS) {
        const uint32_t b = (a + NARROW_MAX_LEVELS < l1) ? a + NARROW_MAX_LEVELS : l1;
        if (mode == MODE_PROVE) {
            if (tiny == 1)
                hipLaunchKernelGGL((k_interp_narrow_b<MODE_PROVE, 0>), dim3(batch), dim3(1024), 0, st, d_gates, d_level_range, a, b, d_pp);
            else
                hipLaunchKernelGGL((k_interp_narrow_b<MODE_PROVE, 64>), dim3(batch), dim3(1024), 0, st, d_gates, d_level_range, a, b, d_pp);
        } else {
            if (tiny == 1)
                hipLaunchKernelGGL((k_interp_narrow_b<MODE_VERIFY, 0>), dim3(batch), dim3(1024), 0, st, d_gates, d_level_range, a, b, d_pp);
            else
                hipLaunchKernelGGL((k_interp_narrow_b<MODE_VERIFY, 64>), dim3(batch), dim3(1024), 0, st, d_gates, d_level_range, a, b, d_pp);
        }
    }
}

}
```

reverie_amd/csrc/shard.inc:

```
struct HostTrace {
    bool on = false;
    std::chrono::steady_clock::time_point t0;
    std::vector<std::pair<const char*, double>> marks;
    void begin() {
        static const bool env = getenv("RV_BATCH_STATS") != nullptr;
        on = env;
        marks.clear();
        t0 = std::chrono::steady_clock::now();
    }
    void mark(const char* what) {
        if (on) marks.emplace_back(what, std::chrono::duration<double, std::milli>(std::chrono::steady_clock::now() - t0).count());
    }
};
static thread_local HostTrace g_ht;

struct EarlyRun {
    const EarlyPlan* plan = nullptr;
    uint8_t* d_ec = nullptr;
    uint8_t* h_ec = nullptr;
    size_t next = 0;
    size_t pumped = 0;
    std::vector<uint8_t> packed;
    uint32_t* box_dev = nullptr;
    volatile uint32_t* box = nullptr;
    uint32_t seq = 0;
    bool ready(size_t k) const {
        const uint32_t v = __atomic_load_n(&box[1], __ATOMIC_ACQUIRE);
        return (v >> 8) == (seq & 0xFFFFFFu) && (v & 0xFFu) > k;
    }
};

struct rv_shard {
    rv_ctx* ctx = nullptr;
    const rv_circuit* c = nullptr;
    uint32_t rep_begin = 0, R = 0, NQ = 0;
    const uint32_t* d_on_quads = nullptr;
    uint32_t n_on_quads = 0;
    uint8_t* d_seeds = nullptr;
    uint8_t* d_keys = nullptr;
    uint8_t* d_rkbytes = nullptr;
    uint32_t* d_rk = nullptr;
    uint32_t* d_masks = nullptr;
    uint32_t* d_rk_c4 = nullptr;
    bool overlap = false;
    uint64_t ov_head = 0;
    uint64_t ov_next = 0, ov_blocks = 0, ov_chunk = 0;
    const uint32_t* ov_keep = nullptr;
    uint8_t* d_wires = nullptr;
    uint32_t* d_on = nullptr;
    uint8_t* d_pre = nullptr;
    uint8_t* d_wit = nullptr;
    uint8_t* d_vclr = nullptr;
    uint64_t* d_masks64 = nullptr;
    uint64_t* d_wmask64 = nullptr;
    uint64_t* d_wcorr64 = nullptr;
    bool z64f = false;
    hipEvent_t ev_sup64 = nullptr;
    std::function<int()> mid64;
    const uint32_t* d_keep64z = nullptr;
    uint64_t* d_v64 = nullptr;
    uint64_t* d_on64 = nullptr;
    uint64_t* d_pre64 = nullptr;
    uint64_t* d_wit64 = nullptr;
    uint8_t* d_keys64 = nullptr;
    uint32_t* d_rk64 = nullptr;
    uint8_t* d_omit64 = nullptr;
    uint32_t* d_cv[2] = {nullptr, nullptr};
    uint32_t* d_cv2[2] = {nullptr, nullptr};
    uint32_t* d_dig = nullptr;
    uint8_t* d_h = nullptr;
    int* d_err = nullptr;
    uint8_t* d_omit = nullptr;
    uint64_t* d_offs = nullptr;
    uint8_t* d_out = nullptr;
    std::vector<void*> extra;
    std::vector<std::pair<uint64_t, hipEvent_t>> mask_chunks;
    hipEvent_t ev_setup = nullptr;
    std::vector<hipEvent_t> misc_events;
    struct EarlyRun* ec = nullptr;
    uint8_t* od_out = nullptr;
    uint32_t od_n_direct = 0;
    int* err_dst_mapped = nullptr;
    bool err_word_sent = false;
    bool keys_deferred = false;
    bool dig64_filled = false;

    void destroy() {
        for (auto& c : mask_chunks) ctx->sync_pool.push_back(c.second);
        mask_chunks.clear();
        for (hipEvent_t e : misc_events) ctx->sync_pool.push_back(e);
        misc_events.clear();
        if (ev_setup) ctx->sync_pool.push_back(ev_setup);
        ev_setup = nullptr;
        void* ps[] = {d_seeds, d_keys, d_rkbytes, d_rk,    d_masks,  d_wires,   d_on,     d_pre,    d_wit,  d_cv[0],
                      d_cv[1], d_dig,  d_h,       d_err,   d_omit,   d_offs,    d_out,    d_masks64, d_wmask64,
                      d_wcorr64, d_on64, d_pre64, d_wit64, d_keys64, d_rk64,    d_omit64, d_vclr, d_v64, d_rk_c4};
        for (void* p : ps) ctx->release(p);
        for (void* p : extra) ctx->release(p);
    }
};

extern "C" void rv_shard_destroy(rv_shard* s) {
    if (!s) return;
    (void)hipStreamSynchronize(s->ctx->stream);
    if (s->ctx->stream2 && (!s->misc_events.empty() || !s->mask_chunks.empty() || s->ev_setup || s->ec)) (void)hipStreamSynchronize(s->ctx->stream2);
    if (s->overlap && s->ctx->stream_m) (void)hipStreamSynchronize(s->ctx->stream_m);
    s->destroy();
    delete s;
}

struct OvTrace {
    std::vector<std::pair<std::string, hipEvent_t>> ev;
    void mark(const char* what, uint64_t n, hipStream_t st) {
        hipEvent_t e = nullptr;
        (void)hipEventCreate(&e);
        (void)hipEventRecord(e, st);
        ev.emplace_back(std::string(what) + " " + std::to_string(n), e);
    }
};
static thread_local OvTrace* g_ov_trace = nullptr;
static void overlap_trace_dump() {
    if (!g_ov_trace) return;
    for (auto& kv : g_ov_trace->ev) {
        float ms = 0;
        (void)hipEventSynchronize(kv.second);
        (void)hipEventElapsedTime(&ms, g_ov_trace->ev[0].second, kv.second);
        fprintf(stderr, "[ov] %9.1f us  %s\n", ms * 1e3, kv.first.c_str());
    }
    for (auto& kv : g_ov_trace->ev) (void)hipEventDestroy(kv.second);
    delete g_ov_trace;
    g_ov_trace = nullptr;
}
static int shard_setup_prg(rv_shard* s, const uint32_t* d_keep, const uint32_t* d_keep64 = nullptr) {
    rv_ctx* ctx = s->ctx;
    const Compiled& cc = s->c->cc;
    int rc;
    const uint64_t n_blocks64 = (cc.n_masks64 + 1) / 2;
    if (n_blocks64) {
        if ((rc = dalloc(ctx, (size_t)n_blocks64 * 2 * s->R * 8, &s->d_masks64))) return rc;
        if (s->d_keys64) {
            if ((rc = dalloc(ctx, (size_t)RK_AREAS * 128 * s->NQ, &s->d_rk64))) return rc;
        }
    }
    if ((rc = dalloc(ctx, (size_t)s->R * 8 * RK_BYTES, &s->d_rkbytes))) return rc;
    if ((rc = dalloc(ctx, (size_t)RK_AREAS * 128 * s->NQ, &s->d_rk))) return rc;
    const uint64_t n_blocks = cc.n_masks_pad / 128;
    if ((rc = dalloc(ctx, (size_t)cc.n_rows * s->NQ, &s->d_masks))) return rc;
    if (!s->keys_deferred) {
        launch_key_schedule(ctx->stream, s->d_keys, s->R * 8, s->d_rkbytes);
        launch_bitslice_rk(ctx->stream, s->d_rkbytes, s->NQ, s->d_rk);
        ctx->count(2);
    }
    static const int col4_mode = [] {
        const char* e = getenv("RV_AES_COL4");
        return e ? atoi(e) : -1;
    }();
    const bool col4 = n_blocks && !g_recorder && aes_col4_supports(s->NQ) && (col4_mode > 0 || (col4_mode < 0 && (s->overlap || n_blocks <= 4096)));
    if (s->overlap && !col4) s->overlap = false;
    if (col4) {
        if ((rc = dalloc(ctx, aes_col4_image_bytes(s->NQ) / 4, &s->d_rk_c4))) return rc;
        if (!s->keys_deferred) {
            launch_rk_col4(ctx->stream, s->d_rk, s->NQ, s->d_rk_c4);
            ctx->count();
        }
    }
    if (s->keys_deferred) {
        launch_setup_keys(ctx->stream, s->d_seeds, s->NQ, s->d_keys, s->d_rkbytes, s->d_rk, col4 ? s->d_rk_c4 : nullptr);
        ctx->count();
    }
    ctx->phase(RV_PH_MASKS);
    if (n_blocks64) {
        const uint32_t* rk64 = s->d_rk;
        if (s->d_keys64) {
            launch_key_schedule(ctx->stream, s->d_keys64, s->R * 8, s->d_rkbytes);
            launch_bitslice_rk(ctx->stream, s->d_rkbytes, s->NQ, s->d_rk64);
            rk64 = s->d_rk64;
        }
        if (s->z64f) {
            s->d_keep64z = s->d_keys64 ? d_keep64 : d_keep;
            for (const auto& run : s->c->z64f_runs) {
                launch_aes_z64_masks(ctx->stream, rk64, s->d_keep64z, s->NQ, run.second, s->d_masks64 + (size_t)run.first * 2 * s->R * 8, run.first);
                ctx->count(1);
            }
        } else {
            launch_aes_z64_masks(ctx->stream, rk64, s->d_keys64 ? d_keep64 : d_keep, s->NQ, n_blocks64, s->d_masks64);
            ctx->count(1);
        }
    }
    if (s->overlap) {
        if (!ctx->stream_m && (ctx->has_prio ? hipStreamCreateWithPriority(&ctx->stream_m, hipStreamNonBlocking, ctx->mask_prio)
                                             : hipStreamCreateWithFlags(&ctx->stream_m, hipStreamNonBlocking)) != hipSuccess)
            return hip_fail(hipGetLastError(), "hipStreamCreate", __FILE__, __LINE__);
        s->ev_setup = ctx->get_sync_event();
        HIPCHK(hipEventRecord(s->ev_setup, ctx->stream));
        HIPCHK(hipStreamWaitEvent(ctx->stream_m, s->ev_setup, 0));
        static const uint64_t n_chunks = [] {
            const char* e = getenv("RV_OVERLAP_CHUNKS");
            return (uint64_t)std::min(std::max(e ? atoi(e) : 16, 1), 256);
        }();
        s->ov_blocks = n_blocks;
        s->ov_chunk = std::max<uint64_t>((n_blocks + n_chunks - 1) / n_chunks, 1024);
        s->ov_keep = d_keep;
        const uint64_t head = std::min(s->ov_head, n_blocks);
        if (head) {
            launch_aes_gf2_masks(ctx->stream, s->d_rk, d_keep, s->NQ, 0, head, s->d_masks);
            ctx->count();
            s->ov_next = head;
        }
        static const bool trace = getenv("RV_OV_TRACE") && atoi(getenv("RV_OV_TRACE")) != 0;
        if (trace) {
            overlap_trace_dump();
            g_ov_trace = new OvTrace();
            g_ov_trace->mark("main: keys done", 0, ctx->stream);
        }
        ctx->phase(-1);
        return RV_OK;
    }
    if (n_blocks) {
        if (col4)
            launch_aes_gf2_masks_col4(ctx->stream, s->d_rk_c4, d_keep, s->NQ, 0, n_blocks, s->d_masks);
        else
            launch_aes_gf2_masks(ctx->stream, s->d_rk, d_keep, s->NQ, 0, n_blocks, s->d_masks);
        ctx->count();
    }
    ctx->phase(-1);
    return RV_OK;
}

static int overlap_need(rv_shard* s, uint64_t need, hipStream_t sb) {
    rv_ctx* ctx = s->ctx;
    need = std::min(need, s->ov_blocks);
    while (s->ov_next < need) {
        if (g_ov_trace) g_ov_trace->mark("main: levels queued so far end; wait for chunk ending at block", s->ov_next, sb);
        if (g_ov_trace) g_ov_trace->mark("  masks: chunk start at block", s->ov_next, ctx->stream_m);
        constexpr uint64_t first = 0;
        const uint64_t nb = std::min(s->ov_next == 0 ? (first ? first : std::max<uint64_t>(s->ov_chunk / 2, 512)) : s->ov_chunk, s->ov_blocks - s->ov_next);
        const auto ht0 = std::chrono::steady_clock::now();
        launch_aes_gf2_masks_col4(ctx->stream_m, s->d_rk_c4, s->ov_keep, s->NQ, s->ov_next, nb, s->d_masks + (size_t)s->ov_next * 128 * s->NQ);
        const auto ht1 = std::chrono::steady_clock::now();
        ctx->count();
        s->ov_next += nb;
        hipEvent_t e = ctx->get_sync_event();
        HIPCHK(hipEventRecord(e, ctx->stream_m));
        const auto ht2 = std::chrono::steady_clock::now();
        s->mask_chunks.emplace_back(s->ov_next, e);
        if (g_ov_trace) g_ov_trace->mark("  masks: chunk end at block", s->ov_next, ctx->stream_m);
        HIPCHK(hipStreamWaitEvent(sb, e, 0));
        if (g_ht.on) {
            const auto ht3 = std::chrono::steady_clock::now();
            auto ms = [](std::chrono::steady_clock::time_point a, std::chrono::steady_clock::time_point b) { return std::chrono::duration<double, std::milli>(b - a).count(); };
            if (ms(ht0, ht1) > 2) g_ht.mark("(slow: chunk launch)");
            if (ms(ht1, ht2) > 2) g_ht.mark("(slow: chunk event record)");
            if (ms(ht2, ht3) > 2) g_ht.mark("(slow: wait event)");
        }
        if (g_ov_trace) g_ov_trace->mark("main: chunk arrived, levels go on; block", s->ov_next, sb);
    }
    return RV_OK;
}

static const uint32_t* b3_empty_digest() {
    static const std::vector<uint32_t> empty = [] {
        b3::Hasher hs;
        uint8_t out[32];
        hs.finalize(out);
        std::vector<uint32_t> w(8);
        for (int k = 0; k < 8; k++) w[k] = (uint32_t)out[4 * k] | ((uint32_t)out[4 * k + 1] << 8) | ((uint32_t)out[4 * k + 2] << 16) | ((uint32_t)out[4 * k + 3] << 24);
        return w;
    }();
    return empty.data();
}

static int shard_run_alloc(rv_shard* s, InterpParams& p, Interp64Params& p64) {
    rv_ctx* ctx = s->ctx;
    const Compiled& cc = s->c->cc;
    int rc;
    if ((rc = dalloc(ctx, (size_t)cc.n_rows * (s->NQ / 2), &s->d_wires))) return rc;
    if ((rc = dalloc(ctx, (size_t)std::max<uint64_t>(cc.n_on, 1) * s->NQ, &s->d_on))) return rc;
    if ((rc = dalloc(ctx, (size_t)std::max<uint64_t>(cc.n_pre, 1) * (s->NQ / 2), &s->d_pre))) return rc;
    if (!s->d_err && (rc = dalloc(ctx, 1, &s->d_err))) return rc;
    const size_t cvw = b3_stream_scratch_words(std::max({cc.n_on, cc.n_pre, cc.on_words64 * 8, cc.pre_words64 * 8}), s->R);
    if ((rc = dalloc(ctx, cvw, &s->d_cv[0])) || (rc = dalloc(ctx, cvw, &s->d_cv[1]))) return rc;
    if (b3_pair_big_ok(cc.n_pre, cc.n_on, s->NQ, s->d_on_quads, s->n_on_quads)) {
        const size_t w2 = b3_stream_scratch_words(std::max(cc.n_on, cc.n_pre), s->R);
        if ((rc = dalloc(ctx, w2, &s->d_cv2[0])) || (rc = dalloc(ctx, w2, &s->d_cv2[1]))) return rc;
        s->extra.push_back(s->d_cv2[0]);
        s->extra.push_back(s->d_cv2[1]);
    }
    if ((rc = dalloc(ctx, (size_t)4 * s->R * 8, &s->d_dig))) return rc;
    if (!s->d_h && (rc = dalloc(ctx, (size_t)s->R * 32, &s->d_h))) return rc;
    const bool has64 = !cc.gates64.empty();
    if (has64) {
        if ((rc = dalloc(ctx, (size_t)cc.n_ssa64 * s->R * 8, &s->d_wmask64))) return rc;
        if (s->z64f && !s->d_keys64) {
            if ((rc = dalloc(ctx, (size_t)cc.n_ssa64, &s->d_v64))) return rc;
            HIPCHK(hipMemsetAsync(s->d_v64, 0, 8, ctx->stream));
        } else {
            if ((rc = dalloc(ctx, (size_t)cc.n_ssa64 * s->R, &s->d_wcorr64))) return rc;
            HIPCHK(rv::memset_async(s->d_wcorr64, 0, (size_t)s->R * 8, ctx->stream));
        }
        if ((rc = dalloc(ctx, (size_t)std::max<uint64_t>(cc.on_words64, 1) * s->R, &s->d_on64))) return rc;
        if ((rc = dalloc(ctx, (size_t)std::max<uint64_t>(cc.pre_words64, 1) * s->R, &s->d_pre64))) return rc;
        HIPCHK(rv::memset_async(s->d_wmask64, 0, (size_t)s->R * 64, ctx->stream));
    }
    hipStream_t sb = ctx->stream;
    s->dig64_filled = !g_recorder && cc.pre_words64 == 0 && cc.on_words64 == 0;
    launch_shard_init(sb, s->d_err, s->d_masks + (size_t)cc.zero_row * s->NQ, s->NQ,
                      s->d_wires + (size_t)cc.zero_row * (s->NQ / 2), s->NQ / 2, s->dig64_filled ? s->d_dig + 2 * (size_t)s->R * 8 : nullptr, 2 * s->R,
                      b3_empty_digest(), p.vclr ? p.vclr + cc.zero_row : nullptr);
    p.NQ = s->NQ;
    p.rows = s->d_masks;
    p.corr = s->d_wires;
    p.on = s->d_on;
    p.pre = s->d_pre;
    p.err = s->d_err;
    p64.R = s->R;
    p64.wmask = s->d_wmask64;
    p64.wcorr = s->d_wcorr64;
    p64.masks = s->d_masks64;
    p64.on = s->d_on64;
    p64.pre = s->d_pre64;
    p64.on_words = cc.on_words64;
    p64.pre_words = cc.pre_words64;
    p64.corr2 = s->d_wires;
    p64.masks2 = s->d_masks;
    p64.NQ = s->NQ;
    p64.err = s->d_err;
    return RV_OK;
}

static bool lds_run_fits_rows(uint32_t qs, uint32_t NQ) { return NQ % qs == 0 && (qs > 1 || NQ % 8 == 0); }

static bool lds_run_for_batch(const rv_circuit* c, size_t level, size_t batch) {
    if (c->lds_run_of_level[level] < 0) return false;
    const auto& pl = c->lds_runs[(size_t)c->lds_run_of_level[level]];
    const size_t limit = getenv("RV_LDS_BATCH_WGS") ? (size_t)atoll(getenv("RV_LDS_BATCH_WGS")) : 768;
    return batch * (RV_TOTAL_REPS / 4 / pl.qs) <= limit;
}

static std::atomic<uint64_t> g_overlap_commits{0};
extern "C" uint64_t rv_hook_overlap_commits(void) { return g_overlap_commits.load(std::memory_order_relaxed); }
static std::atomic<uint64_t> g_early_proofs{0};
extern "C" uint64_t rv_hook_early_proofs(void) { return g_early_proofs.load(std::memory_order_relaxed); }
static std::atomic<uint64_t> g_open_direct_proofs{0};
extern "C" uint64_t rv_hook_open_direct_proofs(void) { return g_open_direct_proofs.load(std::memory_order_relaxed); }
static std::atomic<uint64_t> g_verify_vc{0};
extern "C" uint64_t rv_hook_verify_vc_count(void) { return g_verify_vc.load(std::memory_order_relaxed); }

static void early_plan_build(const rv_circuit* c, EarlyPlan& P) {
    const Compiled& cc = c->cc;
    const uint64_t min_events = getenv("RV_EARLY_MIN") ? (uint64_t)atoll(getenv("RV_EARLY_MIN")) : (1ull << 21);
    const int n_chunks_env = getenv("RV_EARLY_CHUNKS") ? std::min(atoi(getenv("RV_EARLY_CHUNKS")), 255) : 4;
    auto reps_env = [](uint32_t dflt) -> uint32_t {
        const char* e = getenv("RV_EARLY_REPS");
        if (!e) return dflt;
        return (uint32_t)std::min(std::max(atoi(e), 0), (int)RV_TOTAL_REPS);
    };
    const size_t n_levels = cc.level_start.empty() ? 0 : cc.level_start.size() - 1;
    if (!cc.gates64.empty()) {
        const size_t n_lv64 = cc.level_start64.empty() ? 0 : cc.level_start64.size() - 1;
        const uint64_t min64 = getenv("RV_EARLY_MIN") ? min_events : (1ull << 17);
        if (cc.row_prg_base || cc.n_pre || cc.pre_words64 != cc.n_corr64 || cc.n_corr64 < min64 || (cc.n_corr64 & 1) || !n_lv64 || n_chunks_env < 1) return;
        std::vector<uint64_t> lo(n_lv64, UINT64_MAX);
        for (size_t l = 0; l < n_lv64; l++)
            for (uint32_t i = cc.level_start64[l]; i < cc.level_start64[l + 1]; i++) {
                const uint32_t op = cc.gates64[i].op;
                if (op == G64_B2A) return;
                if (op == G64_MUL) lo[l] = std::min<uint64_t>(lo[l], cc.gates64[i].ep);
            }
        std::vector<uint64_t> done(n_lv64);
        uint64_t m = cc.pre_words64;
        for (size_t l = n_lv64; l-- > 0;) {
            done[l] = m;
            m = std::min(m, lo[l]);
        }
        const uint64_t vec_bytes = 8 * cc.n_corr64;
        uint32_t r_spec;
        if (getenv("RV_EARLY") && atoi(getenv("RV_EARLY")) == 2) {
            r_spec = reps_env(128);
        } else {
            const double t_window = (double)cc.gates64.size() * 19e-9 + (double)cc.n_corr64 * 6e-9;
            r_spec = (uint32_t)std::min<double>(RV_TOTAL_REPS, 0.9 * t_window * 55e9 / (double)vec_bytes);
        }
        r_spec = std::min<uint32_t>(r_spec, RV_TOTAL_REPS) & ~7u;
        if (r_spec < 64) return;
        const uint64_t pitch = (vec_bytes + 127) & ~127ull;
        const uint64_t K = getenv("RV_EARLY_CHUNKS") ? (uint64_t)n_chunks_env : 12;
        const uint64_t per = ((vec_bytes + K - 1) / K + 127) & ~127ull;
        for (uint64_t b0 = 0; b0 < vec_bytes; b0 += per) {
            EarlyPlan::Chunk ch{};
            ch.byte0 = b0;
            ch.nbytes = std::min(per, vec_bytes - b0);
            ch.pitch = pitch;
            ch.off = 0;
            const uint64_t need = (ch.byte0 + ch.nbytes) / 8;
            ch.ready_level = (uint32_t)(std::lower_bound(done.begin(), done.end(), need) - done.begin());
            if (ch.ready_level >= n_lv64) return;
            const uint64_t k = P.chunks.size();
            if (ch.ready_level > n_lv64 * (k + 1) / K + n_lv64 / 4) return;
            P.chunks.push_back(ch);
        }
        P.bytes = (size_t)r_spec * pitch;
        P.z64 = true;
        P.r_spec = r_spec;
        P.ok = true;
        return;
    }
    if (cc.row_prg_base || cc.n_pre < min_events || !n_levels || n_chunks_env < 1) return;
    uint32_t r_spec = RV_TOTAL_REPS;
    if (getenv("RV_EARLY") && atoi(getenv("RV_EARLY")) == 2) {
        r_spec = reps_env(RV_TOTAL_REPS);
    } else {
        const bool beside = !(getenv("RV_OVERLAP") && atoi(getenv("RV_OVERLAP")) == 0);
        const double t_levels = std::max({(double)n_levels * 13e-6, (double)cc.gates.size() * 0.25e-9, beside ? (double)(cc.n_masks_pad / 128) * 38e-9 : 0.0});
        const double t_window = t_levels + (double)cc.n_pre * 0.21e-9 + 0.3e-3;
        r_spec = (uint32_t)std::min<double>(RV_TOTAL_REPS, 0.9 * t_window * 55e9 / ((double)cc.n_pre / 8.0));
    }
    r_spec = std::min<uint32_t>(r_spec, RV_TOTAL_REPS) & ~7u;
    if (r_spec < 64) return;
    std::vector<uint64_t> lo(n_levels, UINT64_MAX);
    const int T = std::max(1, std::min<int>(16, (int)std::thread::hardware_concurrency()));
    auto scan = [&](size_t l0, size_t l1) {
        for (size_t l = l0; l < l1; l++) {
            uint64_t m = UINT64_MAX;
            for (uint32_t i = cc.level_start[l]; i < cc.level_start[l + 1]; i++)
                if (g_op(cc.gates[i]) == G_MUL) m = std::min<uint64_t>(m, cc.gates[i].ep);
            lo[l] = m;
        }
    };
    {
        std::vector<std::thread> th;
        size_t l0 = 0;
        for (int t = 0; t < T; t++) {
            const uint32_t want = (uint32_t)((uint64_t)cc.gates.size() * (t + 1) / T);
            size_t l1 = t + 1 == T ? n_levels : (size_t)(std::lower_bound(cc.level_start.begin(), cc.level_start.end(), want) - cc.level_start.begin());
            l1 = std::min(std::max(l1, l0), n_levels);
            if (l1 > l0) {
                if (t + 1 == T) scan(l0, l1); else th.emplace_back(scan, l0, l1);
            }
            l0 = l1;
        }
        for (auto& t : th) t.join();
    }
    std::vector<uint64_t> done(n_levels);
    uint64_t m = cc.n_pre;
    for (size_t l = n_levels; l-- > 0;) {
        done[l] = m;
        m = std::min(m, lo[l]);
    }
    const uint64_t l2c = cc.n_pre / 8 + 1;
    const uint64_t K = (uint64_t)n_chunks_env;
    const uint64_t per = ((l2c + K - 1) / K + 127) & ~127ull;
    size_t off = 0;
    for (uint64_t b0 = 0; b0 < l2c; b0 += per) {
        EarlyPlan::Chunk ch{};
        ch.byte0 = b0;
        ch.nbytes = std::min(per, l2c - b0);
        ch.pitch = (ch.nbytes + 127) & ~127ull;
        ch.off = off;
        off += (size_t)256 * ch.pitch;
        const uint64_t need = std::min<uint64_t>(8 * (ch.byte0 + ch.nbytes), cc.n_pre);
        ch.ready_level = (uint32_t)(std::lower_bound(done.begin(), done.end(), need) - done.begin());
        if (ch.ready_level >= n_levels) return;
        const uint64_t k = P.chunks.size();
        if (ch.ready_level > n_levels * (k + 1) / K + n_levels / 4) return;
        P.chunks.push_back(ch);
    }
    P.bytes = off;
    P.r_spec = r_spec;
    P.ok = true;
}
static const EarlyPlan* early_plan(const rv_circuit* c) {
    std::call_once(c->ec_once, [c] { early_plan_build(c, c->ec_plan); });
    return &c->ec_plan;
}
static uint64_t early_staging_bytes_of(const rv_circuit* c) {
    if (const char* e = getenv("RV_EARLY"))
        if (atoi(e) == 0) return 0;
    EarlyPlan P;
    early_plan_build(c, P);
    return P.ok ? (uint64_t)P.bytes : 0;
}

extern "C" int rv_hook_early_plan(const rv_op* ops, size_t n_ops, size_t z64_wires, size_t gf2_wires, uint32_t flags, uint64_t out[22]) {
    if (!out || (n_ops && !ops) || (flags & ~RV_COMPILE_WHOLE_PROVER)) return RV_E_ARG;
    try {
        rv_circuit tmp;
        int rc = compile_ops(ops, n_ops, z64_wires, gf2_wires, tmp.cc, nullptr, ((flags & RV_COMPILE_WHOLE_PROVER) && !getenv("RV_LAZY_K")) ? RV_LIN_K : 0);
        if (rc) return rc;
        const EarlyPlan* P = early_plan(&tmp);
        for (int i = 0; i < 22; i++) out[i] = 0;
        out[0] = P->ok, out[1] = P->z64, out[2] = P->r_spec, out[3] = P->chunks.size(), out[4] = P->bytes;
        if (!P->ok) return RV_OK;
        const Compiled& cc = tmp.cc;
        bool good = true;
        for (size_t k = 0; k < P->chunks.size(); k++) {
            const auto& ch = P->chunks[k];
            if (k < 16) out[6 + k] = ch.ready_level;
            const uint64_t row0 = P->z64 ? ch.byte0 / 8 : ch.byte0 * 8;
            const uint64_t row1 = P->z64 ? (ch.byte0 + ch.nbytes) / 8 : std::min<uint64_t>((ch.byte0 + ch.nbytes) * 8, cc.n_pre);
            bool at_ready = row1 <= row0;
            const size_t n_levels = (P->z64 ? cc.level_start64.size() : cc.level_start.size()) - 1;
            for (size_t l = 0; l < n_levels; l++) {
                const uint32_t a = P->z64 ? cc.level_start64[l] : cc.level_start[l], b = P->z64 ? cc.level_start64[l + 1] : cc.level_start[l + 1];
                for (uint32_t i = a; i < b; i++) {
                    uint64_t ep;
                    if (P->z64) {
                        if (cc.gates64[i].op != G64_MUL) continue;
                        ep = cc.gates64[i].ep;
                    } else {
                        if (g_op(cc.gates[i]) != G_MUL) continue;
                        ep = cc.gates[i].ep;
                    }
                    if (ep < row1 && l > ch.ready_level) good = false;
                    if (ep >= row0 && ep < row1 && l == ch.ready_level) at_ready = true;
                }
            }
            if (!at_ready && !(k && ch.ready_level == P->chunks[k - 1].ready_level)) good = false;
            if (k && ch.ready_level < P->chunks[k - 1].ready_level) good = false;
            if (k && ch.byte0 != P->chunks[k - 1].byte0 + P->chunks[k - 1].nbytes) good = false;
        }
        out[5] = good;
        return RV_OK;
    } catch (...) {
        g_last_error = "out of host memory";
        return RV_E_NOMEM;
    }
}

static int early_flush_chunks(rv_shard* s, size_t last) {
    EarlyRun* e = s->ec;
    rv_ctx* ctx = s->ctx;
    const auto& chunks = e->plan->chunks;
    if (e->next >= chunks.size() || last <= e->next) return RV_OK;
    constexpr int pack_stream = 1;
    const size_t first = e->next;
    for (size_t k = first; k < last; k++) {
        const bool in_stream = pack_stream == 1 || (pack_stream != 2 && k + 1 == chunks.size());
        const auto& ch = chunks[k];
        if (e->plan->z64) {
            e->packed.push_back(1);
            continue;
        }
        if (in_stream) {
            launch_pack_corr_all(ctx->stream, s->d_pre, s->c->cc.n_pre, ch.byte0, ch.nbytes, ch.pitch, e->d_ec + ch.off);
            if (ctx->profiling) ctx->prof.launches[RV_PH_EARLY]++;
        }
        e->packed.push_back(in_stream ? 1 : 0);
    }
    launch_publish(ctx->stream, nullptr, 0, nullptr, e->box_dev + 1, (e->seq << 8) | (uint32_t)last);
    if (ctx->profiling) ctx->prof.launches[RV_PH_EARLY]++;
    e->next = last;
    return RV_OK;
}
static int early_flush(rv_shard* s, size_t levels_queued) {
    EarlyRun* e = s->ec;
    const auto& chunks = e->plan->chunks;
    if (e->next >= chunks.size() || chunks[e->next].ready_level >= levels_queued) return RV_OK;
    size_t last = e->next;
    while (last < chunks.size() && chunks[last].ready_level < levels_queued) last++;
    return early_flush_chunks(s, last);
}

template <class Pred>
static int mailbox_wait(rv_ctx* ctx, Pred arrived, double* ema_us, const char* what) {
    constexpr bool spin_only = false;
    static const long timeout_ms = getenv("RV_EARLY_TIMEOUT_MS") ? std::max(atol(getenv("RV_EARLY_TIMEOUT_MS")), 1l) : 20000;
    const auto t0 = std::chrono::steady_clock::now();
    auto elapsed_us = [&] { return std::chrono::duration<double, std::micro>(std::chrono::steady_clock::now() - t0).count(); };
    if (!spin_only && ema_us && *ema_us > 200.0) {
        const double until = 0.8 * *ema_us - 80.0;
        while (!arrived()) {
            const double left = until - elapsed_us();
            if (left < 30.0) break;
            timespec ts{0, (long)(std::min(left, 250.0) * 1000.0)};
            nanosleep(&ts, nullptr);
        }
    }
    int rc = RV_OK;
    for (uint64_t spins = 0; !arrived(); spins++) {
        __builtin_ia32_pause();
        if ((spins & 0xFFFF) == 0xFFFF) {
            const hipError_t q = hipStreamQuery(ctx->stream);
            if (q != hipErrorNotReady && !arrived()) {
                rc = q == hipSuccess ? RV_E_DEVICE : hip_fail(q, what, __FILE__, __LINE__);
                break;
            }
            if (elapsed_us() > 1e3 * (double)timeout_ms * 10.0) {
                g_last_error = std::string(what) + ": no word from a still running stream within 10 x RV_EARLY_TIMEOUT_MS (" + std::to_string(10ull * timeout_ms) + " ms)";
                rc = RV_E_DEVICE;
                break;
            }
        }
    }
    if (rc == RV_OK && ema_us) *ema_us = *ema_us > 0 ? 0.7 * *ema_us + 0.3 * elapsed_us() : elapsed_us();
    return rc;
}

static int early_pump(rv_shard* s) {
    EarlyRun* e = s->ec;
    rv_ctx* ctx = s->ctx;
    const auto& chunks = e->plan->chunks;
    for (; e->pumped < chunks.size(); e->pumped++) {
        const size_t k = e->pumped;
        if (k >= e->packed.size()) return RV_E_DEVICE;
        if (int rcw = mailbox_wait(ctx, [&] { return e->ready(k); }, k < 16 ? &ctx->ec_wait_us[k] : nullptr, "early corrections (pump)")) return rcw;
        const auto& ch = chunks[k];
        if (e->plan->z64) {
            HIPCHK(hipMemcpy2DAsync(e->h_ec + ch.byte0, ch.pitch, (const uint8_t*)s->d_pre64 + ch.byte0, (size_t)s->c->cc.pre_words64 * 8, ch.nbytes,
                                    e->plan->r_spec, hipMemcpyDeviceToHost, ctx->stream2));
        } else {
            if (!e->packed[k]) launch_pack_corr_all(ctx->stream2, s->d_pre, s->c->cc.n_pre, ch.byte0, ch.nbytes, ch.pitch, e->d_ec + ch.off);
            HIPCHK(hipMemcpyAsync(e->h_ec + ch.off, e->d_ec + ch.off, (size_t)e->plan->r_spec * ch.pitch, hipMemcpyDeviceToHost, ctx->stream2));
        }
    }
    return RV_OK;
}


static int shard_run_levels(rv_shard* s, int mode, const InterpParams& p, const Interp64Params& p64) {
    rv_ctx* ctx = s->ctx;
    const Compiled& cc = s->c->cc;
    const bool has64 = !cc.gates64.empty();
    hipStream_t sb = ctx->stream;
    const size_t n_levels = cc.level_start.empty() ? 0 : cc.level_start.size() - 1;
    ctx->phase(RV_PH_INTERP, sb);
    size_t waited = 0;
    int rc_ec;
    const uint32_t n_qg64 = s->z64f ? s->NQ / z64_fused_qw(s->NQ) : 0;
    auto fused_params = [&](uint32_t qg0, uint32_t qgn) {
        Z64FParams zp{};
        zp.rk = s->d_keys64 ? s->d_rk64 : s->d_rk;
        zp.NQ = s->NQ;
        zp.wmask = p64.wmask;
        zp.masks = s->d_masks64;
        zp.on = p64.on;
        zp.pre = p64.pre;
        zp.on_words = p64.on_words;
        zp.pre_words = p64.pre_words;
        zp.wit = p64.wit;
        zp.v = s->d_v64;
        zp.err = p64.err;
        zp.first_block = 0;
        zp.qg0 = qg0;
        zp.qgn = qgn;
        if (mode == MODE_VERIFY) {
            zp.omit = p64.omit;
            zp.keep = s->d_keep64z;
            zp.wcorr = p64.wcorr;
            zp.sup_in = p64.sup_in;
            zp.sup_corr = p64.sup_corr;
            zp.sup_rec = p64.sup_rec;
            zp.sup_r = p64.sup_r;
        }
        return zp;
    };
    if (s->z64f && s->ev_sup64 && mode == MODE_VERIFY) {
        for (int pass = 0; pass < 2; pass++) {
            if (pass == 1) {
                int rcm = s->mid64 ? s->mid64() : RV_OK;
                s->mid64 = nullptr;
                if (rcm) return rcm;
                HIPCHK(hipStreamWaitEvent(sb, s->ev_sup64, 0));
            }
            const Z64FParams zp = pass == 0 ? fused_params(1, n_qg64 - 1) : fused_params(0, 1);
            for (size_t l = 0; l < n_levels; l++)
                if (cc.level_start64[l + 1] > cc.level_start64[l]) {
                    launch_z64_fused(sb, s->c->d_gates64f, s->c->z64f_levels[l], zp);
                    ctx->count();
                }
        }
        return RV_OK;
    }
    auto ht_last = std::chrono::steady_clock::now();
    for (size_t l = 0; l < n_levels; l++) {
        if (g_ht.on) {
            const auto now = std::chrono::steady_clock::now();
            if (std::chrono::duration<double, std::milli>(now - ht_last).count() > 2) g_ht.mark("(slow: level iteration)");
            ht_last = now;
        }
        if (s->ec && (rc_ec = early_flush(s, l))) return rc_ec;
        if (s->overlap) {
            size_t l_need = l;
            if (s->c->lds_run_of_level[l] >= 0) l_need = std::max(l_need, (size_t)s->c->lds_runs[(size_t)s->c->lds_run_of_level[l]].run.l1 - 1);
            if (s->c->run_of_level[l] >= 0) l_need = std::max(l_need, (size_t)s->c->narrow_runs[(size_t)s->c->run_of_level[l]].second - 1);
            if ((rc_ec = overlap_need(s, cc.level_need_blocks[l_need], sb))) return rc_ec;
            waited = s->mask_chunks.size();
        }
        while (waited < s->mask_chunks.size() &&
               (waited == 0 ? 0 : s->mask_chunks[waited - 1].first) < cc.level_need_blocks[l]) {
            HIPCHK(hipStreamWaitEvent(sb, s->mask_chunks[waited].second, 0));
            waited++;
        }
        const bool own_launch = mode == MODE_PROVE_V || mode == MODE_VERIFY_C;
        if (!own_launch && s->c->lds_run_of_level[l] >= 0 && lds_run_fits_rows(s->c->lds_runs[(size_t)s->c->lds_run_of_level[l]].qs, p.NQ)) {
            const auto& pl = s->c->lds_runs[(size_t)s->c->lds_run_of_level[l]];
            if (l == pl.run.l0) {
                while (waited < s->mask_chunks.size() &&
                       (waited == 0 ? 0 : s->mask_chunks[waited - 1].first) < cc.level_need_blocks[pl.run.l1 - 1]) {
                    HIPCHK(hipStreamWaitEvent(sb, s->mask_chunks[waited].second, 0));
                    waited++;
                }
                launch_interp_lds(sb, mode, pl.qs, p.NQ, s->c->d_lds_recs + pl.run.rec0, pl.run.n_steps, pl.run.n_slots, pl.run.eo0, pl.run.ep0, p, nullptr, 1);
                ctx->count();
            }
            continue;
        }
        if (s->c->run_of_level[l] >= 0 && !own_launch) {
            const auto& run = s->c->narrow_runs[(size_t)s->c->run_of_level[l]];
            if (l == run.first) {
                while (waited < s->mask_chunks.size() &&
                       (waited == 0 ? 0 : s->mask_chunks[waited - 1].first) < cc.level_need_blocks[run.second - 1]) {
                    HIPCHK(hipStreamWaitEvent(sb, s->mask_chunks[waited].second, 0));
                    waited++;
                }
                launch_interp_narrow(sb, mode, s->c->d_gates, s->c->d_level_range, run.first, run.second, run.tiny, p);
                ctx->count();
            }
            continue;
        }
        if (cc.level_start[l + 1] > cc.level_start[l]) {
            const LevelRange* next = (l + 1 < n_levels && (s->c->run_of_level[l + 1] < 0 || own_launch) && cc.level_start[l + 2] > cc.level_start[l + 1])
                                         ? &cc.level_range[l + 1]
                                         : nullptr;
            launch_interp(sb, mode, s->c->d_gates, cc.level_range[l], p, next);
            ctx->count();
        }
        if (has64 && cc.level_start64[l + 1] > cc.level_start64[l]) {
            if (s->z64f) {
                const Z64FParams zp = fused_params(0, n_qg64);
                    launch_z64_fused(sb, s->c->d_gates64f, s->c->z64f_levels[l], zp);
            } else {
                launch_interp64(sb, mode, s->c->d_gates64, cc.level_start64[l], cc.level_start64[l + 1], p64);
            }
            ctx->count();
        }
    }
    if (s->ec && (rc_ec = early_flush(s, n_levels))) return rc_ec;
    if (s->overlap && (rc_ec = overlap_need(s, s->ov_blocks, sb))) return rc_ec;
    if (s->overlap && mode != MODE_VERIFY && mode != MODE_VERIFY_C) g_overlap_commits.fetch_add(1, std::memory_order_relaxed);
    if (g_ov_trace) g_ov_trace->mark("main: last level done", n_levels, sb);
    return RV_OK;
}

static int shard_run_hash(rv_shard* s) {
    rv_ctx* ctx = s->ctx;
    const Compiled& cc = s->c->cc;
    ctx->phase(RV_PH_HASH);
    uint32_t* dig = s->d_dig;
    const size_t DW = (size_t)s->R * 8;
    uint32_t n_launch;
    constexpr bool pair_on = true;
    if (pair_on && launch_b3_pair_small(ctx->stream, s->d_pre, cc.n_pre, s->d_on, cc.n_on, s->NQ, s->d_cv[0], s->d_cv[1], dig + 0 * DW, dig + 1 * DW,
                                        s->d_on_quads, s->n_on_quads)) {
        n_launch = 2;
    } else if (s->d_cv2[0]) {
        n_launch = launch_b3_pair_big(ctx->stream, s->d_pre, cc.n_pre, s->d_on, cc.n_on, s->NQ, s->d_cv[0], s->d_cv[1], s->d_cv2[0], s->d_cv2[1], dig + 0 * DW, dig + 1 * DW,
                                      s->d_on_quads, s->n_on_quads);
    } else {
        n_launch = launch_b3_stream_bits(ctx->stream, s->d_pre, cc.n_pre, s->NQ, s->d_cv[0], s->d_cv[1], dig + 0 * DW);
        n_launch += launch_b3_stream(ctx->stream, s->d_on, cc.n_on, s->NQ, s->d_cv[0], s->d_cv[1], dig + 1 * DW, s->d_on_quads, s->n_on_quads);
    }
    if (cc.pre_words64 == 0 && cc.on_words64 == 0) {
        if (!s->dig64_filled) {
            launch_fill_digests(ctx->stream, dig + 2 * DW, 2 * s->R, b3_empty_digest());
            n_launch += 1;
        }
    } else {
        n_launch += launch_b3_contig(ctx->stream, s->d_pre64, cc.pre_words64, s->R, s->d_cv[0], s->d_cv[1], dig + 2 * DW);
        n_launch += launch_b3_contig(ctx->stream, s->d_on64, cc.on_words64, s->R, s->d_cv[0], s->d_cv[1], dig + 3 * DW);
    }
    ctx->count(n_launch);
    ctx->phase(-1);
    return RV_OK;
}

static int shard_run(rv_shard* s, int mode, InterpParams& p, Interp64Params& p64) {
    int rc;
    if ((rc = shard_run_alloc(s, p, p64))) return rc;
    g_ht.mark("alloc");
    if ((rc = shard_run_levels(s, mode, p, p64))) return rc;
    g_ht.mark("levels");
    if ((rc = shard_run_hash(s))) return rc;
    g_ht.mark("hash");
    return RV_OK;
}

static int shard_join(rv_shard* s) {
    const size_t DW = (size_t)s->R * 8;
    s->ctx->phase(RV_PH_JOIN);
    s->ctx->count();
    launch_join(s->ctx->stream, s->d_dig, s->d_dig + DW, s->d_dig + 2 * DW, s->d_dig + 3 * DW, s->R, s->d_h);
    s->ctx->phase(-1);
    HIPCHK(hipGetLastError());
    return RV_OK;
}


static int rv_shard_commit_impl(rv_ctx* ctx, const rv_circuit* c, const WitSrc& w, const uint8_t* seeds, uint32_t rep_begin, uint32_t rep_count,
                               rv_shard** out, bool defer_sync = false, EarlyRun* ec = nullptr);

extern "C" int rv_shard_commit(rv_ctx* ctx, const rv_circuit* c, const uint8_t* wit_gf2, size_t n_gf2, const uint64_t* wit_z64,
                               size_t n_z64, const uint8_t* seeds, uint32_t rep_begin, uint32_t rep_count, rv_shard** out) {
    try {
        return rv_shard_commit_impl(ctx, c, wit_host(wit_gf2, n_gf2, wit_z64, n_z64), seeds, rep_begin, rep_count, out);
    } catch (...) {
        g_last_error = "out of host memory";
        return RV_E_NOMEM;
    }
}

static int rv_shard_commit_impl(rv_ctx* ctx, const rv_circuit* c, const WitSrc& w, const uint8_t* seeds, uint32_t rep_begin, uint32_t rep_count,
                               rv_shard** out, bool defer_sync, EarlyRun* ec) {
    LibBusy busy_guard;
    if (!ctx || !c || !out || !seeds) return RV_E_ARG;
    const uint8_t* const wit_gf2 = w.gf2;
    const uint64_t* const wit_z64 = w.z64;
    const size_t n_gf2 = w.n_gf2, n_z64 = w.n_z64;
    if (rep_count == 0 || rep_count % 8 || rep_begin % 8 || rep_begin + rep_count > RV_TOTAL_REPS) return RV_E_ARG;
    *out = nullptr;
    const Compiled& cc = c->cc;
    if (n_gf2 < cc.n_in || n_z64 < cc.n_in64) return RV_E_WITNESS_SHORT;
    if ((cc.n_in && !wit_gf2) || (cc.n_in64 && !wit_z64)) return RV_E_ARG;
    HIPCHK(hipSetDevice(ctx->device));
    rv_shard* s = new rv_shard();
    s->ctx = ctx;
    s->c = c;
    s->rep_begin = rep_begin;
    s->R = rep_count;
    s->NQ = rep_count / 4;
    int rc = RV_OK;
    auto fail = [&](int code) {
        rv_shard_destroy(s);
        return code;
    };
    const size_t seed_bytes = (size_t)s->R * 16;
    const bool stage_in = defer_sync && seed_bytes + cc.n_in <= rv_ctx::IN_STAGE_BYTES &&
                          (ctx->h_in || hipHostMalloc((void**)&ctx->h_in, rv_ctx::IN_STAGE_BYTES, hipHostMallocDefault) == hipSuccess);
    if (!stage_in) (void)hipGetLastError();
    if (stage_in) {
        if ((rc = dalloc(ctx, seed_bytes + std::max<size_t>(cc.n_in, 1), &s->d_seeds)) || (rc = dalloc(ctx, (size_t)s->R * 128, &s->d_keys))) return fail(rc);
        s->d_wit = s->d_seeds + seed_bytes;
        memcpy(ctx->h_in, seeds, seed_bytes);
        const size_t staged_wit = w.dev ? 0 : cc.n_in;
        if (staged_wit) memcpy(ctx->h_in + seed_bytes, wit_gf2, staged_wit);
        if (hipMemcpyAsync(s->d_seeds, ctx->h_in, seed_bytes + staged_wit, hipMemcpyHostToDevice, ctx->stream) != hipSuccess) return fail(RV_E_DEVICE);
        if (w.dev && cc.n_in && hipMemcpyAsync(s->d_wit, wit_gf2, cc.n_in, hipMemcpyDeviceToDevice, ctx->stream) != hipSuccess) return fail(RV_E_DEVICE);
    } else {
        if ((rc = dalloc(ctx, seed_bytes, &s->d_seeds)) || (rc = dalloc(ctx, (size_t)s->R * 128, &s->d_keys)) ||
            (rc = dalloc(ctx, std::max<size_t>(cc.n_in, 1), &s->d_wit)))
            return fail(rc);
        if (hipMemcpyAsync(s->d_seeds, seeds, seed_bytes, hipMemcpyHostToDevice, ctx->stream) != hipSuccess) return fail(RV_E_DEVICE);
        if (cc.n_in && hipMemcpyAsync(s->d_wit, wit_gf2, cc.n_in, w.kind(), ctx->stream) != hipSuccess) return fail(RV_E_DEVICE);
    }
    if (cc.n_in64) {
        if ((rc = dalloc(ctx, cc.n_in64, &s->d_wit64))) return fail(rc);
        if (hipMemcpyAsync(s->d_wit64, wit_z64, cc.n_in64 * 8, w.kind(), ctx->stream) != hipSuccess)
            return fail(RV_E_DEVICE);
    }
    wit_count(w, cc.n_in + cc.n_in64 * 8);
    static const bool vclr_on = [] {
        const char* e = getenv("RV_VCLR");
        return !e || atoi(e) != 0;
    }();
    const bool use_vclr = vclr_on && c->vclr_ok && (s->NQ == 64 || s->NQ == 32 || s->NQ == 16 || s->NQ == 8);
    s->z64f = c->z64f_ok && z64_fused_on() && z64_fused_supports(s->NQ) && !g_recorder;
    {
        const int ov_mode = getenv("RV_OVERLAP") ? atoi(getenv("RV_OVERLAP")) : 1;
        const uint64_t ov_min = getenv("RV_OVERLAP_MIN") ? strtoull(getenv("RV_OVERLAP_MIN"), nullptr, 0) : 8192;
        s->overlap = ov_mode != 0 && !g_recorder && aes_col4_supports(s->NQ) &&
                     cc.n_masks_pad / 128 >= ov_min;
    }
    ctx->phase(RV_PH_SETUP);
    ctx->count();
    s->keys_deferred = !g_recorder && s->R == 4 * s->NQ;
    if (!s->keys_deferred) launch_expand_seeds(ctx->stream, s->d_seeds, s->R, s->d_keys);
    {
        g_ht.mark("inputs");
        if ((rc = shard_setup_prg(s, nullptr))) return fail(rc);
        g_ht.mark("prg");
        if (ec) s->ec = ec;
        InterpParams p{};
        p.wit = s->d_wit;
        Interp64Params p64{};
        p64.wit = s->d_wit64;
        int mode = MODE_PROVE;
        if (use_vclr) {
            if ((rc = dalloc(ctx, (size_t)cc.n_rows, &s->d_vclr))) return fail(rc);
            p.vclr = s->d_vclr;
            mode = MODE_PROVE_V;
        }
        if ((rc = shard_run(s, mode, p, p64))) return fail(rc);
    }
    if ((rc = shard_join(s))) return fail(rc);
    if (defer_sync) {
        ctx->prof.calls++;
        *out = s;
        return RV_OK;
    }
    int err = 0;
    if (hipMemcpyAsync(&err, s->d_err, sizeof err, hipMemcpyDeviceToHost, ctx->stream) != hipSuccess) return fail(RV_E_DEVICE);
    hipError_t e = hipStreamSynchronize(ctx->stream);
    if (e != hipSuccess) {
        hip_fail(e, "hipStreamSynchronize", __FILE__, __LINE__);
        return fail(RV_E_DEVICE);
    }
    ctx->collect();
    ctx->prof.calls++;
    if (err) return fail(RV_E_WITNESS_INVALID);
    *out = s;
    return RV_OK;
}

extern "C" int rv_shard_digests_device(rv_shard* s, void** dptr) {
    if (!s || !dptr) return RV_E_ARG;
    *dptr = s->d_h;
    return RV_OK;
}

extern "C" int rv_shard_digests(rv_shard* s, uint8_t* out) {
    if (!s || !out) return RV_E_ARG;
    HIPCHK(hipMemcpyAsync(out, s->d_h, (size_t)s->R * 32, hipMemcpyDeviceToHost, s->ctx->stream));
    HIPCHK(hipStreamSynchronize(s->ctx->stream));
    return RV_OK;
}

extern "C" int rv_shard_digests_to_device(rv_shard* s, void* dst_device) {
    if (!s || !dst_device) return RV_E_ARG;
    HIPCHK(hipMemcpyAsync(dst_device, s->d_h, (size_t)s->R * 32, hipMemcpyDeviceToDevice, s->ctx->stream));
    HIPCHK(hipStreamSynchronize(s->ctx->stream));
    return RV_OK;
}

extern "C" int rv_hook_shard_stream_digests(rv_shard* s, uint8_t* out) {
    if (!s || !out) return RV_E_ARG;
    std::vector<uint32_t> tmp((size_t)4 * s->R * 8);
    HIPCHK(hipMemcpyAsync(tmp.data(), s->d_dig, tmp.size() * 4, hipMemcpyDeviceToHost, s->ctx->stream));
    HIPCHK(hipStreamSynchronize(s->ctx->stream));
    for (uint32_t r = 0; r < s->R; r++)
        for (int k = 0; k < 4; k++) memcpy(out + ((size_t)r * 4 + k) * 32, &tmp[((size_t)k * s->R + r) * 8], 32);
    return RV_OK;
}
```

Baseline: 985.0 million AND gates/s.

## Process four 32-bit words per lane in NQ=64 prover level interpreter

Adds an x4 variant of the full-width level interpreter in which each lane handles four consecutive row words through 128-bit vector loads and stores, so one wave covers four gates at NQ=64. Gate records are loaded for all gates in the wave and selected per lane, and in PROVE_V mode the pre-share bits are computed from parity bits directly, skipping a smear/compress round trip. It is enabled by default for prover modes when pointers are suitably aligned. In exchange, register pressure per lane rises (launch bounds are set to 6 or 8 waves), and the gate-record select costs extra loads and ALU work.

```diff
diff --git a/reverie_amd/csrc/batch.inc b/reverie_amd/csrc/batch.inc
--- a/reverie_amd/csrc/batch.inc
+++ b/reverie_amd/csrc/batch.inc
@@ -60,6 +60,7 @@
     const Compiled& cc = c->cc;
     const bool has64 = !cc.gates64.empty();
     const size_t n_levels = cc.level_start.empty() ? 0 : cc.level_start.size() - 1;
+    const int x4 = level_x4_from_env();
     for (size_t l = 0; l < n_levels; l++) {
         if (lds_run_for_batch(c, l, batch)) {
             const auto& pl = c->lds_runs[(size_t)c->lds_run_of_level[l]];
@@ -78,7 +79,7 @@
             }
             continue;
         }
-        launch_interp_batched(ctx->stream, c->d_gates, cc.level_range[l], d_pp, (uint32_t)batch, mode);
+        launch_interp_batched(ctx->stream, c->d_gates, cc.level_range[l], d_pp, (uint32_t)batch, mode, x4);
         if (has64 && cc.level_start[l + 1] > cc.level_start[l]) ctx->count();
         if (has64 && cc.level_start64[l + 1] > cc.level_start64[l]) {
             launch_interp64_batched(ctx->stream, mode, c->d_gates64, cc.level_start64[l], cc.level_start64[l + 1], d_pp64, (uint32_t)batch);
diff --git a/reverie_amd/csrc/gf2dev.h b/reverie_amd/csrc/gf2dev.h
--- a/reverie_amd/csrc/gf2dev.h
+++ b/reverie_amd/csrc/gf2dev.h
@@ -16,6 +16,50 @@
     t &= 0x01010101u;
     return smear01(t);
 }
+__device__ __forceinline__ uint32_t parity01(uint32_t t) {
+    t ^= t >> 4;
+    t ^= t >> 2;
+    t ^= t >> 1;
+    return t & 0x01010101u;
+}
+
+struct q4 {
+    uint32_t x, y, z, w;
+};
+typedef uint32_t u32x4 __attribute__((ext_vector_type(4)));
+template <int W>
+struct qwords {
+    using type = uint32_t;
+};
+template <>
+struct qwords<4> {
+    using type = q4;
+};
+__device__ __forceinline__ q4 operator^(q4 a, q4 b) { return q4{a.x ^ b.x, a.y ^ b.y, a.z ^ b.z, a.w ^ b.w}; }
+__device__ __forceinline__ q4 operator&(q4 a, q4 b) { return q4{a.x & b.x, a.y & b.y, a.z & b.z, a.w & b.w}; }
+__device__ __forceinline__ q4& operator^=(q4& a, q4 b) { return a = a ^ b; }
+__device__ __forceinline__ q4 recon32(q4 t) { return q4{recon32(t.x), recon32(t.y), recon32(t.z), recon32(t.w)}; }
+__device__ __forceinline__ q4 parity01(q4 t) { return q4{parity01(t.x), parity01(t.y), parity01(t.z), parity01(t.w)}; }
+__device__ __forceinline__ q4 smear01(q4 t) { return q4{smear01(t.x), smear01(t.y), smear01(t.z), smear01(t.w)}; }
+__device__ __forceinline__ q4 splat01(q4, uint32_t bit) {
+    const uint32_t m = 0u - bit;
+    return q4{m, m, m, m};
+}
+__device__ __forceinline__ uint32_t splat01(uint32_t, uint32_t bit) { return 0u - bit; }
+__device__ __forceinline__ uint32_t ld(const uint32_t* p) { return *p; }
+__device__ __forceinline__ uint32_t ld_nt(const uint32_t* p) { return __builtin_nontemporal_load(p); }
+__device__ __forceinline__ void st(uint32_t* p, uint32_t v) { *p = v; }
+__device__ __forceinline__ void st_nt(uint32_t* p, uint32_t v) { __builtin_nontemporal_store(v, p); }
+__device__ __forceinline__ q4 ld(const q4* p) {
+    const u32x4 v = *(const u32x4*)p;
+    return q4{v.x, v.y, v.z, v.w};
+}
+__device__ __forceinline__ q4 ld_nt(const q4* p) {
+    const u32x4 v = __builtin_nontemporal_load((const u32x4*)p);
+    return q4{v.x, v.y, v.z, v.w};
+}
+__device__ __forceinline__ void st(q4* p, q4 v) { *(u32x4*)p = u32x4{v.x, v.y, v.z, v.w}; }
+__device__ __forceinline__ void st_nt(q4* p, q4 v) { __builtin_nontemporal_store(u32x4{v.x, v.y, v.z, v.w}, (u32x4*)p); }
 
 __device__ __forceinline__ uint32_t expand4(uint32_t n) {
     const uint32_t t = (n | (n << 7) | (n << 14) | (n << 21)) & 0x01010101u;
@@ -36,5 +80,22 @@
     const uint32_t other = pair_swap(n);
     if (!(q & 1)) base[row * (NQ >> 1) + (q >> 1)] = (uint8_t)(n | (other << 4));
 }
+__device__ __forceinline__ uint32_t compress16(q4 x) {
+    return compress4(x.x) | (compress4(x.y) << 4) | (compress4(x.z) << 8) | (compress4(x.w) << 12);
+}
+__device__ __forceinline__ uint32_t compress4_01(uint32_t y) { return (y | (y >> 7) | (y >> 14) | (y >> 21)) & 0xFu; }
+__device__ __forceinline__ uint32_t compress16_01(q4 x) {
+    return compress4_01(x.x) | (compress4_01(x.y) << 4) | (compress4_01(x.z) << 8) | (compress4_01(x.w) << 12);
+}
+__device__ __forceinline__ q4 expand16(uint32_t n) {
+    return q4{expand4(n & 0xFu), expand4((n >> 4) & 0xFu), expand4((n >> 8) & 0xFu), expand4((n >> 12) & 0xFu)};
+}
+__device__ __forceinline__ uint32_t load_bits16(const uint8_t* base, size_t row, uint32_t j) {
+    return *(const uint16_t*)(base + row * 32 + 2 * j);
+}
+__device__ __forceinline__ void store_bits16(uint8_t* base, size_t row, uint32_t j, uint32_t bits) {
+    *(uint16_t*)(base + row * 32 + 2 * j) = (uint16_t)bits;
+}
+__device__ __forceinline__ void store_bits4(uint8_t* base, size_t row, uint32_t j, q4 smeared) { store_bits16(base, row, j, compress16(smeared)); }
 
 }
diff --git a/reverie_amd/csrc/internal.h b/reverie_amd/csrc/internal.h
--- a/reverie_amd/csrc/internal.h
+++ b/reverie_amd/csrc/internal.h
@@ -157,12 +157,13 @@
     uint32_t lo, mul11, mul, xor2, xork, hi;
 };
 bool any_level_general(const LevelRange* lr, size_t n_levels);
+int level_x4_from_env();
 void launch_interp(hipStream_t st, int mode, const Gate* d_gates, const LevelRange& r, const InterpParams& p,
-                   const LevelRange* next = nullptr);
+                   const LevelRange* next = nullptr, int x4 = 0);
 void launch_interp_narrow(hipStream_t st, int mode, const Gate* d_gates, const LevelRange* d_level_range, uint32_t l0, uint32_t l1,
                           int tiny, const InterpParams& p);
 void launch_interp_batched(hipStream_t st, const Gate* d_gates, const LevelRange& r, const InterpParams* d_pp, uint32_t batch,
-                           int mode = MODE_PROVE);
+                           int mode = MODE_PROVE, int x4 = 0);
 bool b3_pair_big_ok(uint64_t n_pre, uint64_t n_on, uint32_t NQ, const uint32_t* d_quads = nullptr, uint32_t n_quads = 0);
 uint32_t launch_b3_pair_big(hipStream_t st, const uint8_t* d_pre, uint64_t n_pre, const uint32_t* d_on, uint64_t n_on, uint32_t NQ, uint32_t* cv_a0,
                             uint32_t* cv_a1, uint32_t* cv_b0, uint32_t* cv_b1, uint32_t* d_dig_pre, uint32_t* d_dig_on, const uint32_t* d_quads = nullptr,
diff --git a/reverie_amd/csrc/interp.hip b/reverie_amd/csrc/interp.hip
--- a/reverie_amd/csrc/interp.hip
+++ b/reverie_amd/csrc/interp.hip
@@ -203,6 +203,15 @@
 #ifndef RV_INTERP_UXOR_FAST
 #define RV_INTERP_UXOR_FAST 0
 #endif
+#ifndef RV_LEVEL_X4_DEFAULT
+#define RV_LEVEL_X4_DEFAULT 1
+#endif
+#ifndef RV_LEVEL_X4_REC
+#define RV_LEVEL_X4_REC 1
+#endif
+#ifndef RV_LEVEL_DELTA_PARITY
+#define RV_LEVEL_DELTA_PARITY 1
+#endif
 __host__ __device__ constexpr int interp_unroll(int NQ, bool general = true) {
     return NQ >= 64 ? (general ? RV_INTERP_UNROLL : RV_INTERP_UNROLL_FAST) : NQ >= 32 ? RV_INTERP_UNROLL_MID : RV_INTERP_UNROLL_SMALL;
 }
@@ -236,43 +245,79 @@
 }
 __device__ __forceinline__ void pf_sink(uint32_t v) { asm volatile("" ::"v"(v)); }
 
-template <int MODE, int NQ, int U, int KA, int KB>
+template <int REC, uint32_t GPW>
+__device__ __forceinline__ Gate load_rec(const Gate* __restrict__ gates, uint32_t g0, uint32_t sub) {
+    if constexpr (REC == 0 || GPW == 1) {
+        return gates[g0 + sub];
+    } else {
+        static_assert(sizeof(Gate) % 4 == 0, "records are selected word by word");
+        constexpr int NW = (int)(sizeof(Gate) / 4);
+        union GW {
+            Gate g;
+            uint32_t w[NW];
+        };
+        GW r[GPW], o;
+#pragma unroll
+        for (uint32_t k = 0; k < GPW; k++) r[k].g = gates[g0 + k];
+#pragma unroll
+        for (int i = 0; i < NW; i++) {
+            uint32_t v = r[0].w[i];
+#pragma unroll
+            for (uint32_t k = 1; k < GPW; k++) v = sub == k ? r[k].w[i] : v;
+            o.w[i] = v;
+        }
+        return o.g;
+    }
+}
+template <int MODE, int NQ, int W>
+__device__ __forceinline__ uint32_t load_cslot(const InterpParams& p, const uint32_t* vc32, uint32_t id, uint32_t q) {
+    if constexpr (MODE == MODE_VERIFY_C) return vc32[2 * (size_t)id];
+    if constexpr (MODE == MODE_PROVE_V) return p.vclr[id];
+    if constexpr (W == 4) return load_bits16(p.corr, id, q);
+    return p.corr[(size_t)id * (NQ / 2) + (q >> 1)];
+}
+
+template <int MODE, int NQ, int U, int KA, int KB, int W = 1, int REC = 0>
 __device__ __forceinline__ void mulU(const Gate* __restrict__ gates, uint32_t g0, const InterpParams& p, uint32_t sub, uint32_t q,
                                      uint32_t onm, const Gate* pf = nullptr) {
-    constexpr uint32_t GPW = 64 / NQ, H = NQ / 2;
+    static_assert(W == 1 || (W == 4 && NQ == 64 && !is_verify(MODE)), "four words per lane: the prover on full-width rows");
+    constexpr uint32_t LPG = NQ / W, GPW = 64 / LPG;
+    using T = typename qwords<W>::type;
+    T* const rows = (T*)p.rows;
+    T* const on = (T*)p.on;
     const bool on_wr = !is_verify(MODE) || ((__ballot(onm != 0) >> ((sub * NQ + q) & ~7u)) & 0xFFull) != 0;
     Gate g[U];
 #pragma unroll
-    for (int u = 0; u < U; u++) g[u] = gates[g0 + u * GPW + sub];
-    uint32_t lx[U], ly[U], lab[U], lnew[U], bx[U], by[U], sc[U], sr[U];
-    uint32_t ra[U][KA], ca[U][KA], rb[U][KB], cb[U][KB];
+    for (int u = 0; u < U; u++) g[u] = load_rec<REC, GPW>(gates, g0 + u * GPW, sub);
+    T lx[U], ly[U], lab[U], lnew[U];
+    uint32_t bx[U], by[U], sc[U], sr[U];
+    T ra[U][KA], rb[U][KB];
+    uint32_t ca[U][KA], cb[U][KB];
     const uint32_t* const vc32 = (const uint32_t*)p.vc + ((q >> 3) & 1u);
 #pragma unroll
     for (int u = 0; u < U; u++) {
         const int na = (int)g_na(g[u]), nb = (int)g_nb(g[u]);
 #pragma unroll
         for (int i = 0; i < KA; i++) {
-            ra[u][i] = 0;
+            ra[u][i] = T();
             ca[u][i] = 0;
             if (i == 0 || i < na) {
-                ra[u][i] = p.rows[(size_t)g[u].a[i] * NQ + q];
-                ca[u][i] = MODE == MODE_VERIFY_C ? vc32[2 * (size_t)g[u].a[i]]
-                                                 : MODE == MODE_PROVE_V ? p.vclr[g[u].a[i]] : p.corr[(size_t)g[u].a[i] * H + (q >> 1)];
+                ra[u][i] = ld(&rows[(size_t)g[u].a[i] * LPG + q]);
+                ca[u][i] = load_cslot<MODE, NQ, W>(p, vc32, g[u].a[i], q);
             }
         }
 #pragma unroll
         for (int i = 0; i < KB; i++) {
-            rb[u][i] = 0;
+            rb[u][i] = T();
             cb[u][i] = 0;
             if (i == 0 || i < nb) {
-                rb[u][i] = p.rows[(size_t)g[u].b[i] * NQ + q];
-                cb[u][i] = MODE == MODE_VERIFY_C ? vc32[2 * (size_t)g[u].b[i]]
-                                                 : MODE == MODE_PROVE_V ? p.vclr[g[u].b[i]] : p.corr[(size_t)g[u].b[i] * H + (q >> 1)];
+                rb[u][i] = ld(&rows[(size_t)g[u].b[i] * LPG + q]);
+                cb[u][i] = load_cslot<MODE, NQ, W>(p, vc32, g[u].b[i], q);
             }
         }
-        lab[u] = __builtin_nontemporal_load(&p.rows[(size_t)g[u].m * NQ + q]);
-        lnew[u] = p.rows[(size_t)(g[u].m + 1) * NQ + q];
-        if (is_verify(MODE)) {
+        lab[u] = ld_nt(&rows[(size_t)g[u].m * LPG + q]);
+        lnew[u] = ld(&rows[(size_t)(g[u].m + 1) * LPG + q]);
+        if constexpr (is_verify(MODE)) {
             sc[u] = sr[u] = 0;
             if (onm) {
                 sc[u] = p.sup_corr[(size_t)g[u].ep * p.sup_nq + q];
@@ -280,7 +325,7 @@
             }
         }
     }
-    const uint32_t pfv = pf_touch<U * GPW>(pf, sub * NQ + q);
+    const uint32_t pfv = pf_touch<U * GPW>(pf, sub * LPG + q);
 #pragma unroll
     for (int u = 0; u < U; u++) {
         lx[u] = ra[u][0];
@@ -300,74 +345,98 @@
     }
 #pragma unroll
     for (int u = 0; u < U; u++) {
-        const uint32_t a = recon32(lx[u]), b = recon32(ly[u]), c = recon32(lab[u]);
-        uint32_t cx, cy;
+        constexpr bool DP = RV_LEVEL_DELTA_PARITY && W == 4 && MODE == MODE_PROVE_V;
+        const T pa = parity01(lx[u]), pb = parity01(ly[u]), pc = parity01(lab[u]);
+        const T a = smear01(pa), b = smear01(pb), c = DP ? T() : smear01(pc);
+        const T ka = splat01(a, g_ca(g[u])), kb = splat01(a, g_cb(g[u]));
+        T cx, cy;
         const uint32_t vx = (bx[u] ^ g_ca(g[u])) & 1u, vy = (by[u] ^ g_cb(g[u])) & 1u;
-        if (MODE == MODE_PROVE_V) {
-            cx = a ^ (vx ? 0xFFFFFFFFu : 0u);
-            cy = b ^ (vy ? 0xFFFFFFFFu : 0u);
-        } else if (MODE == MODE_VERIFY_C) {
-            cx = expand4(q < 16 ? (bx[u] >> (4 * (q & 7))) & 0xFu : 0u) ^ (g_ca(g[u]) ? 0xFFFFFFFFu : 0u);
-            cy = expand4(q < 16 ? (by[u] >> (4 * (q & 7))) & 0xFu : 0u) ^ (g_cb(g[u]) ? 0xFFFFFFFFu : 0u);
-        } else {
-            cx = expand4((bx[u] >> (4 * (q & 1))) & 0xFu) ^ (g_ca(g[u]) ? 0xFFFFFFFFu : 0u);
-            cy = expand4((by[u] >> (4 * (q & 1))) & 0xFu) ^ (g_cb(g[u]) ? 0xFFFFFFFFu : 0u);
-        }
-        uint32_t delta = (a & b) ^ c;
-        uint32_t s = (ly[u] & cx) ^ (lx[u] & cy) ^ lab[u] ^ lnew[u];
-        uint32_t r = 0;
-        if (MODE == MODE_PROVE) {
+        if constexpr (MODE == MODE_PROVE_V) {
+            cx = a ^ splat01(a, vx);
+            cy = b ^ splat01(a, vy);
+        } else if constexpr (MODE == MODE_VERIFY_C) {
+            cx = expand4(q < 16 ? (bx[u] >> (4 * (q & 7))) & 0xFu : 0u) ^ ka;
+            cy = expand4(q < 16 ? (by[u] >> (4 * (q & 7))) & 0xFu : 0u) ^ kb;
+        } else if constexpr (W == 4) {
+            cx = expand16(bx[u]) ^ ka;
+            cy = expand16(by[u]) ^ kb;
+        } else {
+            cx = expand4((bx[u] >> (4 * (q & 1))) & 0xFu) ^ ka;
+            cy = expand4((by[u] >> (4 * (q & 1))) & 0xFu) ^ kb;
+        }
+        T delta = (a & b) ^ c;
+        T s = (ly[u] & cx) ^ (lx[u] & cy) ^ lab[u] ^ lnew[u];
+        T r = T();
+        if constexpr (MODE == MODE_PROVE) {
             r = recon32(s);
-        } else if (is_verify(MODE)) {
+        } else if constexpr (is_verify(MODE)) {
             delta = (sc[u] & onm) | (delta & ~onm);
             s ^= sr[u];
             r = recon32(s) & onm;
         }
-        if (!is_verify(MODE) || on_wr) __builtin_nontemporal_store(s, &p.on[(size_t)g[u].eo * NQ + q]);
-        store_bits(p.pre, g[u].ep, NQ, q, delta);
-        if (MODE == MODE_PROVE_V) {
+        if (!is_verify(MODE) || on_wr) st_nt(&on[(size_t)g[u].eo * LPG + q], s);
+        if constexpr (DP) {
+            store_bits16(p.pre, g[u].ep, q, compress16_01((pa & pb) ^ pc));
             if (q == 0) p.vclr[g[u].dst] = (uint8_t)(vx & vy);
-        } else if (MODE == MODE_VERIFY_C) {
-            vc_store(p.vc, g[u].dst, q, r ^ delta ^ (cx & cy));
-        } else {
-            store_bits(p.corr, g[u].dst, NQ, q, r ^ delta ^ (cx & cy));
+        } else if constexpr (W == 4) {
+            store_bits4(p.pre, g[u].ep, q, delta);
+            if constexpr (MODE == MODE_PROVE_V) {
+                if (q == 0) p.vclr[g[u].dst] = (uint8_t)(vx & vy);
+            } else {
+                store_bits4(p.corr, g[u].dst, q, r ^ delta ^ (cx & cy));
+            }
+        } else {
+            store_bits(p.pre, g[u].ep, NQ, q, delta);
+            if constexpr (MODE == MODE_PROVE_V) {
+                if (q == 0) p.vclr[g[u].dst] = (uint8_t)(vx & vy);
+            } else if constexpr (MODE == MODE_VERIFY_C) {
+                vc_store(p.vc, g[u].dst, q, r ^ delta ^ (cx & cy));
+            } else {
+                store_bits(p.corr, g[u].dst, NQ, q, r ^ delta ^ (cx & cy));
+            }
         }
     }
     pf_sink(pfv);
 }
 
-template <int MODE, int NQ, int U, int N>
+template <int MODE, int NQ, int U, int N, int W = 1, int REC = 0>
 __device__ __forceinline__ void xorU(const Gate* __restrict__ gates, uint32_t g0, const InterpParams& p, uint32_t sub, uint32_t q,
                                      const Gate* pf = nullptr) {
-    constexpr uint32_t GPW = 64 / NQ, H = NQ / 2;
+    static_assert(W == 1 || (W == 4 && NQ == 64 && !is_verify(MODE)), "four words per lane: the prover on full-width rows");
+    constexpr uint32_t LPG = NQ / W, GPW = 64 / LPG, H = NQ / 2;
+    using T = typename qwords<W>::type;
+    T* const rows = (T*)p.rows;
     Gate g[U];
 #pragma unroll
-    for (int u = 0; u < U; u++) g[u] = gates[g0 + u * GPW + sub];
-    uint32_t x[U], bx[U], rr[U][N], cc[U][N];
+    for (int u = 0; u < U; u++) g[u] = load_rec<REC, GPW>(gates, g0 + u * GPW, sub);
+    T x[U], rr[U][N];
+    uint32_t bx[U], cc[U][N];
 #pragma unroll
     for (int u = 0; u < U; u++) {
         const int na = (int)g_na(g[u]), nb = (int)g_nb(g[u]);
 #pragma unroll
         for (int i = 0; i < N; i++) {
             const uint32_t id = (N == 2) ? g[u].a[i] : (i < RV_LIN_K ? g[u].a[i] : g[u].b[i - RV_LIN_K]);
-            rr[u][i] = 0;
+            rr[u][i] = T();
             cc[u][i] = 0;
             if (N == 2 || (i < RV_LIN_K ? i < na : i - RV_LIN_K < nb)) {
-                rr[u][i] = p.rows[(size_t)id * NQ + q];
-                if (MODE == MODE_PROVE_V) {
+                rr[u][i] = ld(&rows[(size_t)id * LPG + q]);
+                if constexpr (MODE == MODE_PROVE_V) {
                     if (q == 0) cc[u][i] = p.vclr[id];
-                } else if (MODE == MODE_VERIFY_C) {
+                } else if constexpr (MODE == MODE_VERIFY_C) {
                     if (q < 2) cc[u][i] = ((const uint32_t*)p.vc)[2 * (size_t)id + q];
+                } else if constexpr (W == 4) {
+                    cc[u][i] = load_bits16(p.corr, id, q);
                 } else if (q < H) {
                     cc[u][i] = p.corr[(size_t)id * H + q];
                 }
             }
         }
     }
-    const uint32_t pfv = pf_touch<U * GPW>(pf, sub * NQ + q);
+    const uint32_t pfv = pf_touch<U * GPW>(pf, sub * LPG + q);
 #pragma unroll
     for (int u = 0; u < U; u++) {
-        x[u] = 0;
+        x[u] = T();
         bx[u] = 0;
 #pragma unroll
         for (int i = 0; i < N; i++) {
@@ -377,11 +446,13 @@
     }
 #pragma unroll
     for (int u = 0; u < U; u++) {
-        p.rows[(size_t)g[u].dst * NQ + q] = x[u];
-        if (MODE == MODE_PROVE_V) {
+        st(&rows[(size_t)g[u].dst * LPG + q], x[u]);
+        if constexpr (MODE == MODE_PROVE_V) {
             if (q == 0) p.vclr[g[u].dst] = (uint8_t)((bx[u] ^ g_ca(g[u])) & 1u);
-        } else if (MODE == MODE_VERIFY_C) {
+        } else if constexpr (MODE == MODE_VERIFY_C) {
             if (q < 2) ((uint32_t*)p.vc)[2 * (size_t)g[u].dst + q] = bx[u] ^ (g_ca(g[u]) ? 0xFFFFFFFFu : 0u);
+        } else if constexpr (W == 4) {
+            store_bits16(p.corr, g[u].dst, q, bx[u] ^ (g_ca(g[u]) ? 0xFFFFu : 0u));
         } else if (q < H) {
             p.corr[(size_t)g[u].dst * H + q] = (uint8_t)(bx[u] ^ (g_ca(g[u]) ? 0xFFu : 0u));
         }
@@ -389,14 +460,17 @@
     pf_sink(pfv);
 }
 
-template <int MODE, int NQ, bool GENERAL = true, bool PF = false, int UXOR = 0>
+template <int MODE, int NQ, bool GENERAL = true, bool PF = false, int UXOR = 0, int W = 1, int REC = 0>
 __device__ __forceinline__ void run_level(const Gate* __restrict__ gates, const LevelRange& r, const InterpParams& p, uint32_t wave,
                                           uint32_t n_waves, uint32_t lane, uint32_t onm, const Gate* pf_gates = nullptr,
                                           const PfPlan* pf = nullptr) {
     constexpr uint32_t GPW = 64 / NQ;
     const uint32_t q = lane % NQ, sub = lane / NQ;
-    constexpr int U = interp_unroll(NQ, GENERAL);
-    constexpr int UX = UXOR ? UXOR : U;
+    static_assert(interp_unroll(NQ, GENERAL) % W == 0 && UXOR % W == 0, "a step is a whole number of W-gate groups");
+    constexpr uint32_t GPS = GPW * W;
+    const uint32_t qs = lane % (NQ / W), subs = lane / (NQ / W);
+    constexpr int U = interp_unroll(NQ, GENERAL) / W;
+    constexpr int UX = UXOR ? UXOR / W : U;
     static_assert(!PF || UX == U, "the prefetch plan assumes one step size");
     uint32_t slot = 0;
     auto my = [&](uint32_t used) { return (wave + n_waves - used % n_waves) % n_waves; };
@@ -404,16 +478,16 @@
     uint32_t rest[5];
 #pragma unroll
     for (int c = 0; c < 4; c++) {
-        const uint32_t STEP = (uint32_t)(c >= 2 ? UX : U) * GPW;
+        const uint32_t STEP = (uint32_t)(c >= 2 ? UX : U) * GPS;
         const uint32_t n_full = (!GENERAL && (c == 1 || c == 3)) ? 0u : (end[c] - begin[c]) / STEP;
         rest[c] = begin[c] + n_full * STEP;
         for (uint32_t g0 = begin[c] + my(slot) * STEP; g0 < rest[c]; g0 += n_waves * STEP) {
             const Gate* t = nullptr;
-            if (PF && pf->dist) t = pf_target<U * GPW>(pf_gates, *pf, slot + (g0 - begin[c]) / STEP);
-            if (c == 0) mulU<MODE, NQ, U, 1, 1>(gates, g0, p, sub, q, onm, t);
-            if (c == 1 && GENERAL) mulU<MODE, NQ, U, RV_LIN_K, RV_LIN_K>(gates, g0, p, sub, q, onm, t);
-            if (c == 2) xorU<MODE, NQ, UX, 2>(gates, g0, p, sub, q, t);
-            if (c == 3 && GENERAL) xorU<MODE, NQ, UX, 2 * RV_LIN_K>(gates, g0, p, sub, q, t);
+            if (PF && pf->dist) t = pf_target<U * GPS>(pf_gates, *pf, slot + (g0 - begin[c]) / STEP);
+            if (c == 0) mulU<MODE, NQ, U, 1, 1, W, REC>(gates, g0, p, subs, qs, onm, t);
+            if (c == 1 && GENERAL) mulU<MODE, NQ, U, RV_LIN_K, RV_LIN_K, W, REC>(gates, g0, p, subs, qs, onm, t);
+            if (c == 2) xorU<MODE, NQ, UX, 2, W, REC>(gates, g0, p, subs, qs, t);
+            if (c == 3 && GENERAL) xorU<MODE, NQ, UX, 2 * RV_LIN_K, W, REC>(gates, g0, p, subs, qs, t);
         }
         slot += n_full;
     }
@@ -444,14 +518,32 @@
     run_level<MODE, NQ, GENERAL, PFL, UXL>(gates, r, p, wave, n_waves, lane, onm, gates, &pf);
 }
 
-template <int MODE, int NQ>
-__global__ __launch_bounds__(256) void k_interp_full_b(const Gate* __restrict__ gates, LevelRange r, const InterpParams* __restrict__ pp) {
+template <int MODE, bool GENERAL, int REC>
+__global__ __launch_bounds__(256, GENERAL ? 6 : 8) void k_interp_full_x4(const Gate* __restrict__ gates, LevelRange r, InterpParams p, PfPlan pf) {
+    static_assert(MODE == MODE_PROVE || MODE == MODE_PROVE_V, "the verify modes' sector logic is keyed by quad word");
+    __builtin_amdgcn_s_setprio(1);
+    const uint32_t lane = threadIdx.x & 63;
+    const uint32_t wave = __builtin_amdgcn_readfirstlane((blockIdx.x * blockDim.x + threadIdx.x) >> 6);
+    const uint32_t n_waves = gridDim.x * (blockDim.x >> 6);
+    constexpr int UXL = !GENERAL ? RV_INTERP_UXOR_FAST : 0;
+    constexpr bool PFL = UXL == 0 || UXL == interp_unroll(64, GENERAL);
+    run_level<MODE, 64, GENERAL, PFL, UXL, 4, REC>(gates, r, p, wave, n_waves, lane, 0u, gates, &pf);
+}
+
+template <int MODE, int NQ, int W = 1, int REC = 0>
+__global__ __launch_bounds__(256, W == 4 ? 6 : 1) void k_interp_full_b(const Gate* __restrict__ gates, LevelRange r, const InterpParams* __restrict__ pp) {
     const InterpParams p = pp[blockIdx.y];
     const uint32_t lane = threadIdx.x & 63;
     const uint32_t wave = __builtin_amdgcn_readfirstlane((blockIdx.x * blockDim.x + threadIdx.x) >> 6);
     const uint32_t n_waves = gridDim.x * (blockDim.x >> 6);
     const uint32_t onm = (is_verify(MODE)) ? p.on_mask[lane % NQ] : 0u;
-    run_level<MODE, NQ>(gates, r, p, wave, n_waves, lane, onm);
+    run_level<MODE, NQ, true, false, 0, W, REC>(gates, r, p, wave, n_waves, lane, onm);
+}
+
+int level_x4_from_env() {
+    const char* e = getenv("RV_LEVEL_X4");
+    if (!e || !*e) return RV_LEVEL_X4_DEFAULT;
+    return atoi(e);
 }
 
 static bool level_is_general(const LevelRange& r) { return (r.mul - r.mul11) + (r.xork - r.xor2) >= 64; }
@@ -491,7 +583,17 @@
 
 template <int MODE, int NQ>
 static void launch_interp_full_mode(hipStream_t st, dim3 grid, bool general, const Gate* d_gates, const LevelRange& r, const InterpParams& p,
-                                    const PfPlan& pf) {
+                                    const PfPlan& pf, int x4 = 0) {
+    if constexpr (NQ == 64 && (MODE == MODE_PROVE || MODE == MODE_PROVE_V)) {
+        if (x4 && ((((uintptr_t)p.rows | (uintptr_t)p.on) & 15) || (((uintptr_t)p.corr | (uintptr_t)p.pre) & 1))) x4 = 0;
+        if (x4) {
+            if (general)
+                hipLaunchKernelGGL((k_interp_full_x4<MODE, true, RV_LEVEL_X4_REC>), grid, dim3(256), 0, st, d_gates, r, p, pf);
+            else
+                hipLaunchKernelGGL((k_interp_full_x4<MODE, false, RV_LEVEL_X4_REC>), grid, dim3(256), 0, st, d_gates, r, p, pf);
+            return;
+        }
+    }
     if (general)
         hipLaunchKernelGGL((k_interp_full<MODE, NQ, true>), grid, dim3(256), 0, st, d_gates, r, p, pf);
     else
@@ -500,7 +602,7 @@
 
 template <int NQ>
 static void launch_interp_full(hipStream_t st, int mode, const Gate* d_gates, const LevelRange& r, const InterpParams& p,
-                               const LevelRange* next) {
+                               const LevelRange* next, int x4) {
     constexpr uint32_t GPW = 64 / NQ;
     const bool general = level_is_general(r);
     const PfPlan pf = make_pf_plan<NQ>(r, next);
@@ -510,8 +612,8 @@
     if (blocks > 4096) blocks = 4096;
     if (blocks < 1) blocks = 1;
     const dim3 grid((unsigned)blocks);
-    if (mode == MODE_PROVE_V) return launch_interp_full_mode<MODE_PROVE_V, NQ>(st, grid, general, d_gates, r, p, pf);
-    if (mode == MODE_PROVE) return launch_interp_full_mode<MODE_PROVE, NQ>(st, grid, general, d_gates, r, p, pf);
+    if (mode == MODE_PROVE_V) return launch_interp_full_mode<MODE_PROVE_V, NQ>(st, grid, general, d_gates, r, p, pf, x4);
+    if (mode == MODE_PROVE) return launch_interp_full_mode<MODE_PROVE, NQ>(st, grid, general, d_gates, r, p, pf, x4);
     if constexpr (NQ == 64)
         if (mode == MODE_VERIFY_C) return launch_interp_full_mode<MODE_VERIFY_C, NQ>(st, grid, general, d_gates, r, p, pf);
     launch_interp_full_mode<MODE_VERIFY, NQ>(st, grid, general, d_gates, r, p, pf);
@@ -607,13 +709,13 @@
     }
 }
 
-void launch_interp(hipStream_t st, int mode, const Gate* d_gates, const LevelRange& r, const InterpParams& p, const LevelRange* next) {
+void launch_interp(hipStream_t st, int mode, const Gate* d_gates, const LevelRange& r, const InterpParams& p, const LevelRange* next, int x4) {
     if (r.hi <= r.lo) return;
     switch (p.NQ) {
-    case 64: return launch_interp_full<64>(st, mode, d_gates, r, p, next);
-    case 32: return launch_interp_full<32>(st, mode, d_gates, r, p, next);
-    case 16: return launch_interp_full<16>(st, mode, d_gates, r, p, next);
-    case 8: return launch_interp_full<8>(st, mode, d_gates, r, p, next);
+    case 64: return launch_interp_full<64>(st, mode, d_gates, r, p, next, x4);
+    case 32: return launch_interp_full<32>(st, mode, d_gates, r, p, next, 0);
+    case 16: return launch_interp_full<16>(st, mode, d_gates, r, p, next, 0);
+    case 8: return launch_interp_full<8>(st, mode, d_gates, r, p, next, 0);
     default: break;
     }
     const uint64_t want = (uint64_t)(r.hi - r.lo) * p.NQ;
@@ -625,13 +727,15 @@
         hipLaunchKernelGGL(k_interp<MODE_VERIFY>, dim3((unsigned)blocks), dim3(256), 0, st, d_gates, r.lo, r.hi, p);
 }
 
-void launch_interp_batched(hipStream_t st, const Gate* d_gates, const LevelRange& r, const InterpParams* d_pp, uint32_t batch, int mode) {
+void launch_interp_batched(hipStream_t st, const Gate* d_gates, const LevelRange& r, const InterpParams* d_pp, uint32_t batch, int mode, int x4) {
     if (r.hi <= r.lo || !batch) return;
     uint64_t waves = ((uint64_t)(r.hi - r.lo) + RV_INTERP_UNROLL - 1) / RV_INTERP_UNROLL;
     uint64_t blocks = (waves + 3) / 4;
     const uint64_t cap = std::max<uint64_t>(4096 / batch, 1);
     if (blocks > cap) blocks = cap;
-    if (mode == MODE_PROVE)
+    if (mode == MODE_PROVE && x4)
+        hipLaunchKernelGGL((k_interp_full_b<MODE_PROVE, 64, 4, RV_LEVEL_X4_REC>), dim3((unsigned)blocks, batch), dim3(256), 0, st, d_gates, r, d_pp);
+    else if (mode == MODE_PROVE)
         hipLaunchKernelGGL((k_interp_full_b<MODE_PROVE, 64>), dim3((unsigned)blocks, batch), dim3(256), 0, st, d_gates, r, d_pp);
     else
         hipLaunchKernelGGL((k_interp_full_b<MODE_VERIFY, 64>), dim3((unsigned)blocks, batch), dim3(256), 0, st, d_gates, r, d_pp);
diff --git a/reverie_amd/csrc/shard.inc b/reverie_amd/csrc/shard.inc
--- a/reverie_amd/csrc/shard.inc
+++ b/reverie_amd/csrc/shard.inc
@@ -672,6 +672,7 @@
         return RV_OK;
     }
     auto ht_last = std::chrono::steady_clock::now();
+    const int x4 = level_x4_from_env();
     for (size_t l = 0; l < n_levels; l++) {
         if (g_ht.on) {
             const auto now = std::chrono::steady_clock::now();
@@ -722,7 +723,7 @@
             const LevelRange* next = (l + 1 < n_levels && (s->c->run_of_level[l + 1] < 0 || own_launch) && cc.level_start[l + 2] > cc.level_start[l + 1])
                                          ? &cc.level_range[l + 1]
                                          : nullptr;
-            launch_interp(sb, mode, s->c->d_gates, cc.level_range[l], p, next);
+            launch_interp(sb, mode, s->c->d_gates, cc.level_range[l], p, next, x4);
             ctx->count();
         }
         if (has64 && cc.level_start64[l + 1] > cc.level_start64[l]) {
@@ -858,7 +859,7 @@
             return fail(RV_E_DEVICE);
     }
     wit_count(w, cc.n_in + cc.n_in64 * 8);
-    static const bool vclr_on = [] {
+    const bool vclr_on = [] {
         const char* e = getenv("RV_VCLR");
         return !e || atoi(e) != 0;
     }();
```

Result: faster. 1.001 billion AND gates/s, median of 6 (+1.6%).
